# reidprichard/ORC

Measured on AMD Instinct MI355X. Metric: SIMPLE iterations/s (10.24M-cell hex channel equivalents; = iterations/s at N=1), higher is better.
Workload: dtype f64

## Files before the change

include/orc_amd.h:

```cpp
#ifndef ORC_AMD_H
#define ORC_AMD_H

#include <stdint.h>
#include "orc_types.h"

#ifdef __cplusplus
extern "C" {
#endif

typedef struct OrcMesh OrcMesh;
typedef struct OrcSolver OrcSolver;

int orc_init(int device_ordinal);
int orc_device_count(void);
int orc_synchronize(void);
const char *orc_status_string(int status);
const char *orc_last_error(void);
int orc_reload_environment(void);
int orc_device_memory(int64_t *free_bytes, int64_t *total_bytes);
int orc_device_info(char *buf, int cap);
void orc_settings_default(OrcSettings *s);

OrcMesh *orc_mesh_create(int64_t n_cells, int64_t n_faces, int32_t n_zones,
                         const int64_t *face_c0, const int64_t *face_c1, const int32_t *face_zone,
                         const double *face_area, const double *face_normal , const double *face_centroid ,
                         const double *cell_centroid , const double *cell_volume,
                         const int64_t *cell_face_ptr , const int64_t *cell_faces,
                         const int32_t *zone_type, const double *zone_scalar, const double *zone_vector ,
                         int *status);
OrcMesh *orc_mesh_create_reordered(int64_t n_cells, int64_t n_faces, int32_t n_zones,
                                   const int64_t *face_c0, const int64_t *face_c1, const int32_t *face_zone,
                                   const double *face_area, const double *face_normal, const double *face_centroid,
                                   const double *cell_centroid, const double *cell_volume,
                                   const int64_t *cell_face_ptr, const int64_t *cell_faces,
                                   const int32_t *zone_type, const double *zone_scalar, const double *zone_vector,
                                   int32_t ordering, int *status);
int orc_mesh_cell_order(const OrcMesh *m, int64_t *global_ids );
OrcMesh *orc_mesh_create_partitioned(int64_t n_owned, int64_t n_cells, int64_t n_cells_global, int64_t n_faces, int32_t n_zones,
                                     const int64_t *face_c0, const int64_t *face_c1, const int32_t *face_zone, const double *face_area,
                                     const double *face_normal, const double *face_centroid, const double *cell_centroid,
                                     const double *cell_volume, const int64_t *cell_face_ptr, const int64_t *cell_faces,
                                     const int32_t *zone_type, const double *zone_scalar, const double *zone_vector, int32_t n_peers,
                                     const int32_t *peers, const int64_t *send_ptr, const int64_t *send_idx, const int64_t *recv_ptr,
                                     int *status);
int64_t orc_mesh_n_owned(const OrcMesh *m);
typedef struct OrcPartition OrcPartition;
OrcPartition *orc_mesh_partition(int64_t n_cells, int64_t n_faces, const int64_t *face_c0, const int64_t *face_c1, const int32_t *face_zone,
                                 const double *face_area, const double *face_normal, const double *face_centroid,
                                 const double *cell_centroid, const double *cell_volume, const int64_t *cell_face_ptr,
                                 const int64_t *cell_faces, int32_t n_ranks, int32_t rank, int32_t ordering, int *status);
OrcPartition *orc_mesh_partition_owner(int64_t n_cells, int64_t n_faces, const int64_t *face_c0, const int64_t *face_c1, const int32_t *face_zone,
                                       const double *face_area, const double *face_normal, const double *face_centroid,
                                       const double *cell_centroid, const double *cell_volume, const int64_t *cell_face_ptr,
                                       const int64_t *cell_faces, const int32_t *cell_owner, int32_t n_ranks, int32_t rank, int64_t n_global,
                                       int *status);
void orc_partition_destroy(OrcPartition *p);
int orc_partition_sizes(const OrcPartition *p, int64_t *n_owned, int64_t *n_local, int64_t *n_global, int64_t *n_faces, int64_t *n_cell_faces,
                        int32_t *n_peers, int64_t *n_send);
int orc_partition_arrays(const OrcPartition *p, int64_t *face_c0, int64_t *face_c1, int32_t *face_zone, double *face_area, double *face_normal,
                         double *face_centroid, double *cell_centroid, double *cell_volume, int64_t *cell_face_ptr, int64_t *cell_faces,
                         int64_t *global_ids, int64_t *global_face_ids, int32_t *peers, int64_t *send_ptr, int64_t *send_idx, int64_t *recv_ptr);
OrcMesh *orc_partition_upload(const OrcPartition *p, int32_t n_zones, const int32_t *zone_type, const double *zone_scalar,
                              const double *zone_vector, int *status);
int orc_mesh_update_zones(OrcMesh *m, const int32_t *zone_type, const double *zone_scalar, const double *zone_vector);
void orc_mesh_destroy(OrcMesh *m);
int64_t orc_mesh_n_cells(const OrcMesh *m);
int64_t orc_mesh_nnz(const OrcMesh *m);
int orc_mesh_matrix_pattern(const OrcMesh *m, int64_t *row_ptr , int64_t *col_idx );

typedef struct OrcMeshData OrcMeshData;
OrcMeshData *orc_read_mesh(const char *mesh_path, int *status);
void orc_mesh_data_destroy(OrcMeshData *d);
int orc_mesh_data_sizes(const OrcMeshData *d, int32_t *dimensions, int64_t *n_vertices, int64_t *n_cells, int64_t *n_faces,
                        int64_t *n_cell_faces, int64_t *n_face_nodes, int32_t *n_zones);
int orc_mesh_data_arrays(const OrcMeshData *d, int64_t *face_c0, int64_t *face_c1, int32_t *face_zone, double *face_area,
                         double *face_normal, double *face_centroid, double *cell_centroid, double *cell_volume,
                         int64_t *cell_face_ptr, int64_t *cell_faces);
int orc_mesh_data_nodes(const OrcMeshData *d, double *vertices , int64_t *face_node_ptr , int64_t *face_nodes);
int orc_mesh_data_zone(const OrcMeshData *d, int32_t k, uint64_t *zone_id, int32_t *zone_type, double *scalar_value,
                       double *vector_value , char *name, int64_t name_len);
int orc_mesh_data_zone_index(const OrcMeshData *d, const char *name);
int orc_mesh_data_set_zone(OrcMeshData *d, const char *name, int32_t zone_type, double scalar_value, const double *vector_value );
OrcMesh *orc_mesh_upload(const OrcMeshData *d, int *status);
int orc_mesh_sync_zones(OrcMesh *m, const OrcMeshData *d);

int orc_write_data(const char *output_file_name, int64_t n_cells, const double *cell_centroid , const double *u,
                   const double *v, const double *w, const double *p, int decimal_precision);
int orc_read_data(const char *data_file_path, int64_t capacity, double *u, double *v, double *w, double *p, int64_t *n_read);
int orc_write_gradients(const OrcMesh *m, const double *cell_centroid, const double *u, const double *v, const double *w,
                        const double *p, const char *output_file_name, int decimal_precision, const OrcSettings *settings);

int orc_iterative_solve(int64_t n, const int64_t *row_ptr, const int64_t *col_idx, const double *values,
                        const double *b, double *solution_vector , uint64_t iteration_count,
                        int method , double relaxation_factor, double convergence_threshold,
                        int preconditioner );
int orc_iterative_solve3(int64_t n, const int64_t *row_ptr, const int64_t *col_idx, const double *const values[3],
                         const double *const b[3], double *const solution_vectors[3] , uint64_t iteration_count,
                         int method, double relaxation_factor, double convergence_threshold, int preconditioner,
                         int status_out[3]);
int orc_set_breakdown_guard(int on);
int64_t orc_breakdown_guard_events(int reset);
int orc_set_reduction_order(int order);
int64_t orc_last_jacobi_sweeps(void);
int orc_set_gmres_restart(int m);
int orc_last_gmres_stats(int64_t *steps, int64_t *cycles, double *initial_residual, double *final_estimate);
int orc_csr_spmv(int64_t n, const int64_t *row_ptr, const int64_t *col_idx, const double *values, const double *x,
                 double *y, int reps, double *avg_ms);

int orc_amg_coarsen(int64_t n, const int64_t *row_ptr, const int64_t *col_idx, const double *values, int64_t *partner ,
                    int64_t *out_n_coarse, int64_t *out_nnz, int64_t *out_row_ptr, int64_t *out_col, double *out_val,
                    int *rounds);

int orc_debug_coloring(int64_t n, const int64_t *row_ptr, const int64_t *col_idx, int32_t *colors , int32_t *n_colors);

int orc_build_momentum_diffusion_matrix(const OrcMesh *m, int diffusion_scheme, double mu,
                                        double *a_values , double *b_u, double *b_v, double *b_w);
int orc_initialize_momentum_matrix(const OrcMesh *m, double *a_values );
int orc_build_momentum_advection_matrices(const OrcMesh *m, double *a_u_values, double *a_v_values, double *a_w_values,
                                          double *b_u, double *b_v, double *b_w, const double *a_di_values,
                                          const double *u, const double *v, const double *w, const double *p,
                                          const OrcSettings *settings, double rho, double peclet[3]);
int orc_build_pressure_correction_matrices(const OrcMesh *m, const double *u, const double *v, const double *w,
                                           const double *p, const double *a_u_values, const double *a_v_values,
                                           const double *a_w_values, const OrcSettings *settings, double rho,
                                           double *a_values , double *b );

int orc_calculate_gradients(const OrcMesh *m, const double *u, const double *v, const double *w, const double *p,
                            const OrcSettings *settings, double *grad_p, double *grad_u);
int orc_check_boundary_conditions(const OrcMesh *m, int *constraint_type);
int orc_initialize_pressure_field(const OrcMesh *m, double *p );
int orc_initialize_flow(const OrcMesh *m, double mu, double rho, uint64_t iteration_count, const OrcSettings *settings,
                        double *u, double *v, double *w, double *p);
int orc_initialize_velocity_field(const OrcMesh *m, const OrcSettings *settings, double *u, double *v, double *w, double *psi);
int orc_initialize_flow_new(const OrcMesh *m, double mu, double rho, uint64_t iteration_count,
                            double *u, double *v, double *w, double *p);
typedef void (*OrcReportFn)(uint64_t iteration, const double mean_velocity[3], const double peclet[3],
                            double velocity_correction, double pressure_correction, double ms_per_iter, void *user);
int orc_solve_steady(OrcMesh *m, double *u, double *v, double *w, double *p, const OrcSettings *settings,
                     double rho, double mu, uint64_t iteration_count, uint64_t reporting_interval,
                     OrcReportFn report_cb, void *user);

OrcSolver *orc_solver_create(OrcMesh *m, const OrcSettings *settings, double rho, double mu, int *status);
void orc_solver_destroy(OrcSolver *s);
int orc_solver_set_fields(OrcSolver *s, const double *u, const double *v, const double *w, const double *p);
int orc_solver_get_fields(OrcSolver *s, double *u, double *v, double *w, double *p);
int orc_solver_iterate(OrcSolver *s, uint64_t iterations, double *report);
int orc_solver_snapshot(OrcSolver *s);
int orc_solver_restore(OrcSolver *s);
int orc_solver_assemble_momentum(OrcSolver *s, double *a_u, double *a_v, double *a_w, double *b_u, double *b_v, double *b_w, double peclet[3]);
int orc_solver_assemble_pressure(OrcSolver *s, double *a_p, double *b_p);

int orc_bench_spmv(OrcSolver *s, int reps, double *avg_ms, double *checksum);
int orc_bench_bicgstab_iteration(OrcSolver *s, int reps, double *avg_ms);
int orc_bench_inloop_products(OrcSolver *s, int reps, double avg_ms[4]);
const char *orc_bench_inloop_variant(void);
int orc_bench_gs_sweep(OrcSolver *s, int reps, double *avg_ms, int *n_colors);
int orc_bench_gs_sweep0(OrcSolver *s, int reps, double avg_ms[2], int *n_colors);
int orc_bench_amg_levels(OrcSolver *s, int reps, int64_t *rows, int64_t *nnz, int64_t *padded, double *avg_ms, int *n_levels);
long long orc_debug_halo_overlaps(void);
int orc_debug_stream_report(char *buf, int cap);
int orc_debug_amg_coarse_product(int64_t n, const int64_t *row_ptr, const int64_t *col_idx, const double *values, int scaled, const double *x,
                                 double *y, int *has_window_mirror);
long long orc_debug_collectives(int reset);
int orc_debug_clamp_partials_grid(long long requested);
int orc_debug_max_partials(void);
int orc_debug_amg_certification(long long out[2], int reset);
int orc_debug_xwin_counters(long long out[3], int reset);
long long orc_debug_shared_galerkin(int reset);
int orc_profile_enable(int on);
int orc_profile_report(char *buf, int64_t buf_len);

int orc_hex_channel_sizes(int64_t nx, int64_t ny, int64_t nz, int64_t *n_cells, int64_t *n_faces, int64_t *n_cell_faces);
int orc_hex_channel_generate(int64_t nx, int64_t ny, int64_t nz, double lx, double ly, double lz,
                             int64_t *face_c0, int64_t *face_c1, int32_t *face_zone, double *face_area,
                             double *face_normal, double *face_centroid, double *cell_centroid, double *cell_volume,
                             int64_t *cell_face_ptr, int64_t *cell_faces);
int orc_hex_channel_write_msh(const char *path, int64_t nx, int64_t ny, int64_t nz, double lx, double ly, double lz);

int orc_mixed_channel_write_msh(const char *path, int64_t nx, int64_t ny, int64_t nz, double lx, double ly, double lz,
                                int64_t *n_cells, int64_t *n_faces);
int orc_poly_channel_write_msh(const char *path, int64_t nx, int64_t ny, int64_t nz, double lx, double ly, double lz,
                               int64_t *n_cells, int64_t *n_faces);
OrcMeshData *orc_mixed_channel_generate(int64_t nx, int64_t ny, int64_t nz, double lx, double ly, double lz, int polyhedra, int *status);

#define ORC_COMM_ID_BYTES 128
int orc_comm_get_unique_id(unsigned char id[ORC_COMM_ID_BYTES]);
int orc_comm_init(const unsigned char id[ORC_COMM_ID_BYTES], int rank, int world_size);
int orc_comm_finalize(void);
int orc_comm_selftest(void);
int orc_comm_init_self_loop(void);
int orc_comm_set_host_transport(void *exchange_fn, void *allreduce_fn, void *user);

#ifdef __cplusplus
}
#endif
#endif
```

orc_amd/csrc/amg.hip:

```cpp
#include <algorithm>
#include <array>
#include <atomic>
#include <chrono>
#include <cmath>
#include <mutex>

#include <thread>

#include "linalg_kernels.hpp"

namespace orc {


__device__ __forceinline__ int64_t sell_pos(const SellDev &P, int64_t row, int k) { return P.slice_ptr[row >> 6] + (int64_t)k * 64 + (row & 63); }

struct AggCounters {
    int changed;
    int rounds;
};

__global__ void agg_reset_k(int *__restrict__ taken_by, int64_t n) {
    for (int64_t i = (int64_t)blockIdx.x * blockDim.x + threadIdx.x; i < n; i += (int64_t)gridDim.x * blockDim.x) taken_by[i] = 0x7fffffff;
}
__global__ void agg_scatter_k(const int *__restrict__ choice, int *__restrict__ taken_by, int64_t n) {
// ... 361 lines not shown
            const int a = (e >= b1) + (e >= b2) + (e >= b3);
            const int c = src_col[e];
            const int own_base = a == 0 ? 0 : (a == 1 ? b1 : (a == 2 ? b2 : b3));
            int rank = e - own_base;
            if (a != 0 && b1 > 0) rank += lds_upper_bound(src_col, b1, c);
            if (a != 1 && b2 > b1) rank += a > 1 ? lds_upper_bound(src_col + b1, b2 - b1, c) : lds_lower_bound(src_col + b1, b2 - b1, c);
            if (a != 2 && b3 > b2) rank += a > 2 ? lds_upper_bound(src_col + b2, b3 - b2, c) : lds_lower_bound(src_col + b2, b3 - b2, c);
            if (a != 3 && b4 > b3) rank += lds_lower_bound(src_col + b3, b4 - b3, c);
            m_col[rank] = c;
            m_val[rank] = src_val[e];
#pragma unroll
            for (int x = 0; x < kX; ++x) x_m[(size_t)x * h + rank] = x_src[(size_t)x * h + e];
        }
        __syncthreads();
        int cntT = 0;
        for (int b0 = 0; b0 < cnt; b0 += G) {
            const int e = b0 + lane;
            int head = 0;
            if (e < cnt) head = (e == 0) || (m_col[e] != m_col[e - 1]);
            int tot;
            const int slot = cntT + group_excl_scan<G>(head, tot);
            if (head) {
                const int j = m_col[e];
                double acc = 0. + m_val[e];
                double xacc[kX > 0 ? kX : 1];
#pragma unroll
                for (int x = 0; x < kX; ++x) xacc[x] = 0. + x_m[(size_t)x * h + e];
                for (int q = e + 1; q < cnt && m_col[q] == j; ++q) {
                    acc += m_val[q];
#pragma unroll
                    for (int x = 0; x < kX; ++x) xacc[x] += x_m[(size_t)x * h + q];
                }
                src_col[slot] = j;
                src_val[slot] = acc;
#pragma unroll
                for (int x = 0; x < kX; ++x) x_src[(size_t)x * h + slot] = xacc[x];
            }
            cntT += tot;
        }
        __syncthreads();
        const int pair0_n = (active_n && 2 * I_n < n_fine) ? choice[2 * I_n] : -1;
        const int pair1_n = (active_n && 2 * I_n + 1 < n_fine) ? choice[2 * I_n + 1] : -1;
        const int *tj = src_col;
        const double *tv = src_val;
        int nU = 0;
        for (int b0 = 0; b0 < cntT; b0 += G) {
            const int e = b0 + lane;
            int k0 = -1, k1 = -1;
            if (e < cntT) {
                const int j = tj[e];
                const int cj = choice[j], mj = chooser[j];
                if (cj >= 0) {
                    const bool dup = (j & 1) && e > 0 && tj[e - 1] == j - 1 && choice[j - 1] >= 0;
                    if (!dup) k0 = j >> 1;
                }
                if (mj >= 0) {
                    const int Jp = mj >> 1;
                    bool drop = cj >= 0 && Jp == (j >> 1);
                    if (!drop) {
                        const int p = lds_lower_bound(tj, cntT, 2 * Jp);
                        const bool has_even = p < cntT && tj[p] == 2 * Jp;
                        if (has_even && choice[2 * Jp] >= 0) drop = true;
                        else {
                            const int q = has_even ? p + 1 : p;
                            if (q < cntT && tj[q] == 2 * Jp + 1 && choice[2 * Jp + 1] >= 0) drop = true;
                        }
                    }
                    if (!drop) {
                        const int sib = mj ^ 1;
                        if (sib < n_fine) {
                            const int js = choice[sib];
                            if (js >= 0 && js < j) {
                                const int p = lds_lower_bound(tj, cntT, js);
                                if (p < cntT && tj[p] == js) drop = true;
                            }
                        }
                    }
                    if (!drop) k1 = Jp;
                }
            }
            int tot;
            int slot = nU + group_excl_scan<G>((k0 >= 0 ? 1 : 0) + (k1 >= 0 ? 1 : 0), tot);
            if (k0 >= 0) U[slot++] = k0;
            if (k1 >= 0) U[slot] = k1;
            nU += tot;
        }
        __syncthreads();
        const long long off = active ? slice_base[I >> 6] + intra_off[I] : 0;
        for (int e = lane; e < nU; e += G) {
            const int u = U[e];
            int rank = 0;
            for (int q = 0; q < nU; ++q) rank += U[q] < u ? 1 : 0;
            const RRow RJ = restriction_row(choice, u, A.P.n);
            double acc = 0.;
            double xacc[kX > 0 ? kX : 1];
#pragma unroll
            for (int x = 0; x < kX; ++x) xacc[x] = 0.;
#pragma unroll
            for (int a = 0; a < 4; ++a) {
                if (a < RJ.n) {
                    const int p = lds_lower_bound(tj, cntT, RJ.idx[a]);
                    if (p < cntT && tj[p] == RJ.idx[a]) {
                        acc += tv[p] * RJ.w[a];
#pragma unroll
                        for (int x = 0; x < kX; ++x) xacc[x] += x_src[(size_t)x * h + p] * RJ.w[a];
                    }
                }
            }
            s_col[off + rank] = u;
            s_val[off + rank] = acc;
#pragma unroll
            for (int x = 0; x < kX; ++x) X.s_val[x][off + rank] = xacc[x];
        }
        if (active && lane == 0) row_len_c[I] = nU;
        __syncthreads();
        active = active_n; I = I_n; pair0 = pair0_n; pair1 = pair1_n;
    }
}

constexpr int kPackDepth = 16;
template <bool kValuesOnly = false>
__global__ __launch_bounds__(64) void galerkin_pack_fused_k(SellDev Pc, const long long *__restrict__ slice_base, const int *__restrict__ intra_off,
                                                            const int *__restrict__ s_col, const double *__restrict__ s_val, int *__restrict__ col_c,
                                                            double *__restrict__ val_c, int *__restrict__ diag_c, const int64_t *__restrict__ pk_ptr,
                                                            int *__restrict__ pk_col, double *__restrict__ pk_val) {
    __shared__ int t_col[kPackDepth * 65];
    __shared__ double t_val[kPackDepth * 65];
    const int lane = threadIdx.x;
    const int kk = lane & (kPackDepth - 1), rr = lane / kPackDepth;
    for (int64_t slice = blockIdx.x; slice < Pc.n_slices; slice += gridDim.x) {
        const int64_t I = slice * 64 + lane;
        const bool live = I < Pc.n;
        const int len = live ? Pc.row_len[I] : 0;
        const long long src = live ? slice_base[slice] + intra_off[I] : 0;
        const int src_lo = (int)(unsigned)(src & 0xffffffffll), src_hi = (int)(src >> 32);
        const int64_t base = Pc.slice_ptr[slice];
        const int width = (int)((Pc.slice_ptr[slice + 1] - base) >> 6);
        int64_t pk_off = pk_ptr ? pk_ptr[slice] : 0;
        int d = -1;
        for (int kc = 0; kc < width; kc += kPackDepth) {
#pragma unroll 4
            for (int rb = 0; rb < 64 / (64 / kPackDepth); ++rb) {
                const int row = rb * (64 / kPackDepth) + rr;
                const int rlen = __shfl(len, row, 64);
                const long long rsrc = ((long long)__shfl(src_hi, row, 64) << 32) | (long long)(unsigned)__shfl(src_lo, row, 64);
                const int k = kc + kk;
                if (k < rlen) {
                    if (!kValuesOnly) t_col[kk * 65 + row] = s_col[rsrc + k];
                    t_val[kk * 65 + row] = s_val[rsrc + k];
                }
            }
            __syncthreads();
            const int kend = min(kPackDepth, width - kc);
            for (int q = 0; q < kend; ++q) {
                const int k = kc + q;
                const bool in = k < len;
                const int c = (in && !kValuesOnly) ? t_col[q * 65 + lane] : (int)I;
                const double v = in ? t_val[q * 65 + lane] : 0.;
                const int64_t pos = base + (int64_t)k * 64 + lane;
                if (live) {
                    if (!kValuesOnly) col_c[pos] = c;
                    val_c[pos] = v;
                    if (!kValuesOnly && in && c == (int)I) d = (int)pos;
                }
                if (pk_ptr) {
                    const unsigned long long m = __ballot(in);
                    const int rank = __builtin_amdgcn_mbcnt_hi((unsigned)(m >> 32), __builtin_amdgcn_mbcnt_lo((unsigned)m, 0u));
                    if (in) {
                        if (!kValuesOnly) pk_col[pk_off + rank] = c;
                        pk_val[pk_off + rank] = v;
                    }
                    pk_off += __popcll(m);
                }
            }
            __syncthreads();
        }
        if (live && !kValuesOnly) diag_c[I] = d;
    }
}

constexpr int kGalerkinTiers = 7;
constexpr int kBoundIters = 32;
__global__ __launch_bounds__(64) void galerkin_bound_k(SellDev P, const int *__restrict__ choice, int64_t n_coarse, int *__restrict__ out_max,
                                                       unsigned long long *__restrict__ out_sum, int *__restrict__ intra_off,
                                                       long long *__restrict__ slice_tot, int *__restrict__ tier_count, int *__restrict__ tier_list, int min_tier) {
    __shared__ signed char tiers[kBoundIters][64];
    const int lane = threadIdx.x;
    const int64_t n_slices = (n_coarse + 63) / 64;
    int mx = 0;
    unsigned long long sm = 0;
    int cnt[kGalerkinTiers];
#pragma unroll
    for (int t = 0; t < kGalerkinTiers; ++t) cnt[t] = 0;
    const int64_t per_wave = (n_slices + gridDim.x - 1) / gridDim.x;
    const int64_t s_lo = (int64_t)blockIdx.x * per_wave, s_hi = s_lo + per_wave < n_slices ? s_lo + per_wave : n_slices;
    int it = 0;
    for (int64_t s = s_lo; s < s_hi && it < kBoundIters; ++s, ++it) {
        const int64_t I = s * 64 + lane;
        int c = 0;
        if (I < n_coarse) {
            const RRow R = restriction_row(choice, I, P.n);
#pragma unroll
            for (int a = 0; a < 4; ++a)
                if (a < R.n) c += P.row_len[R.idx[a]];
        }
        int tot;
        const int ex = wave_excl_scan(2 * c, tot);
        if (I < n_coarse) intra_off[I] = ex;
        if (lane == 0) slice_tot[s] = tot;
        mx = max(mx, c);
        sm += (unsigned long long)c;
        int tier = -1;
        if (I < n_coarse) {
            tier = min_tier;
            while (tier < kGalerkinTiers - 1 && (64 << tier) < 2 * c) ++tier;
        }
        tiers[it][lane] = (signed char)tier;
#pragma unroll
        for (int t = 0; t < kGalerkinTiers; ++t) cnt[t] += __popcll(__ballot(tier == t));
    }
    int base[kGalerkinTiers];
#pragma unroll
    for (int t = 0; t < kGalerkinTiers; ++t) {
        base[t] = 0;
        if (cnt[t] > 0) {
            if (lane == 0) base[t] = atomicAdd(&tier_count[t], cnt[t]);
            base[t] = __shfl(base[t], 0, 64);
        }
    }
    it = 0;
    for (int64_t s = s_lo; s < s_hi && it < kBoundIters; ++s, ++it) {
        const int64_t I = s * 64 + lane;
        const int tier = tiers[it][lane];
#pragma unroll
        for (int t = 0; t < kGalerkinTiers; ++t) {
            const unsigned long long m = __ballot(tier == t);
            if (m == 0ull) continue;
            if (tier == t) tier_list[(int64_t)t * n_coarse + base[t] + __popcll(m & ((1ull << lane) - 1ull))] = (int)I;
            base[t] += __popcll(m);
        }
    }
#pragma unroll
    for (int off = 32; off > 0; off >>= 1) {
        mx = max(mx, __shfl_down(mx, off, 64));
        sm += __shfl_down(sm, off, 64);
    }
    if (lane == 0) { atomicMax(out_max, mx); atomicAdd(out_sum, sm); }
}

constexpr int kScanThreads = 256;
__device__ __forceinline__ long long block_excl_scan(long long v, long long *buf , long long &total) {
    const int t = threadIdx.x;
    buf[t] = v;
    __syncthreads();
    for (int off = 1; off < kScanThreads; off <<= 1) {
        const long long x = t >= off ? buf[t - off] : 0;
        __syncthreads();
        buf[t] += x;
        __syncthreads();
    }
    total = buf[kScanThreads - 1];
    const long long r = buf[t] - v;
    __syncthreads();
    return r;
}

__global__ __launch_bounds__(kBlock) void slice_sizes_k(const int *__restrict__ row_len, int64_t n, int n_slices, int64_t *__restrict__ w_sell,
                                                        int64_t *__restrict__ w_pk) {
    const int lane = threadIdx.x & 63;
    const int64_t wave = ((int64_t)blockIdx.x * blockDim.x + threadIdx.x) >> 6, waves = ((int64_t)gridDim.x * blockDim.x) >> 6;
    for (int64_t s = wave; s < n_slices; s += waves) {
        const int64_t r = s * 64 + lane;
        const int len = r < n ? row_len[r] : 0;
        int mx = len, sum = len;
#pragma unroll
        for (int off = 32; off > 0; off >>= 1) {
            mx = max(mx, __shfl_xor(mx, off, 64));
            sum += __shfl_xor(sum, off, 64);
        }
        if (lane == 0) { w_sell[s] = (int64_t)mx * 64; w_pk[s] = ((int64_t)sum + 15) & ~(int64_t)15; }
    }
}
constexpr int kScanBlocks = 128;
__global__ __launch_bounds__(kScanThreads) void scan_part_k(const long long *__restrict__ in_a, const long long *__restrict__ in_b, int64_t n, int64_t chunk,
                                                            long long *__restrict__ part ) {
    __shared__ long long buf[kScanThreads];
    const int64_t lo = (int64_t)blockIdx.x * chunk, hi = std::min<int64_t>(n, lo + chunk);
    long long sa = 0, sb = 0;
    for (int64_t e = lo + threadIdx.x; e < hi; e += kScanThreads) { sa += in_a[e]; if (in_b) sb += in_b[e]; }
    long long ta, tb;
    (void)block_excl_scan(sa, buf, ta);
    (void)block_excl_scan(sb, buf, tb);
    if (threadIdx.x == 0) { part[blockIdx.x] = ta; part[kScanBlocks + blockIdx.x] = tb; }
}
__global__ __launch_bounds__(kScanThreads) void scan_mid_k(long long *__restrict__ part, int n_blocks) {
    __shared__ long long buf[kScanThreads];
    const int t = threadIdx.x;
    const long long va = t < n_blocks ? part[t] : 0, vb = t < n_blocks ? part[kScanBlocks + t] : 0;
    long long ta, tb;
    const long long ra = block_excl_scan(va, buf, ta);
    const long long rb = block_excl_scan(vb, buf, tb);
    if (t < n_blocks) { part[t] = ra; part[kScanBlocks + t] = rb; }
    if (t == 0) { part[2 * kScanBlocks] = ta; part[2 * kScanBlocks + 1] = tb; }
}
__global__ __launch_bounds__(kScanThreads) void scan_write_k(const long long *__restrict__ in_a, const long long *__restrict__ in_b, int64_t n, int64_t chunk,
                                                             const long long *__restrict__ part, long long *__restrict__ out_a, long long *__restrict__ out_b,
                                                             int write_totals ) {
    __shared__ long long buf[kScanThreads];
    const int64_t lo = (int64_t)blockIdx.x * chunk, hi = std::min<int64_t>(n, lo + chunk);
    long long base_a = part[blockIdx.x], base_b = part[kScanBlocks + blockIdx.x];
    for (int64_t t0 = lo; t0 < hi; t0 += kScanThreads) {
        const int64_t e = t0 + threadIdx.x;
        const long long va = e < hi ? in_a[e] : 0, vb = (in_b && e < hi) ? in_b[e] : 0;
        long long ta, tb = 0;
        const long long ra = block_excl_scan(va, buf, ta);
        long long rb = 0;
        if (in_b) rb = block_excl_scan(vb, buf, tb);
        if (e < hi) { out_a[e] = base_a + ra; if (in_b) out_b[e] = base_b + rb; }
        base_a += ta;
        base_b += tb;
    }
    if (write_totals && blockIdx.x == 0 && threadIdx.x == 0) { out_a[n] = part[2 * kScanBlocks]; if (in_b) out_b[n] = part[2 * kScanBlocks + 1]; }
}
static int scan_excl_dev(const long long *in_a, const long long *in_b, int64_t n, long long *out_a, long long *out_b, bool write_totals, long long *part, hipStream_t st) {
    const int64_t n1 = std::max<int64_t>(n, 1);
    int64_t chunk = (n1 + kScanBlocks - 1) / kScanBlocks;
    chunk = ((chunk + kScanThreads - 1) / kScanThreads) * kScanThreads;
    const int n_blocks = (int)((n1 + chunk - 1) / chunk);
    hipLaunchKernelGGL(scan_part_k, dim3(n_blocks), dim3(kScanThreads), 0, st, in_a, in_b, n, chunk, part);
    hipLaunchKernelGGL(scan_mid_k, dim3(1), dim3(kScanThreads), 0, st, part, n_blocks);
    hipLaunchKernelGGL(scan_write_k, dim3(n_blocks), dim3(kScanThreads), 0, st, in_a, in_b, n, chunk, (const long long *)part, out_a, out_b, write_totals ? 1 : 0);
    ORC_HIP(hipGetLastError());
    return ORC_OK;
}


constexpr int kXBitWords = 8192;
__device__ unsigned long long g_xwin_counters[3];
constexpr int kXBitWordsSmall = 4096;
template <int kWords, bool kSecond>
__global__ __launch_bounds__(kBlock) void xwin_build_k(SellDev P, PackedDev pk, int *__restrict__ wcol, int *__restrict__ wsize,
                                                       unsigned short *__restrict__ lidx, int64_t n_blocks, int win_cap, int bit_words, int pass_words,
                                                       int *__restrict__ pending ) {
    if (kSecond && *pending == 0) return;
    __shared__ unsigned bits[kWords];
    __shared__ unsigned short wpre[kWords];
    __shared__ int s_min, s_max, s_part[kBlock];
    const int tid = threadIdx.x, lane = tid & 63, wave = tid >> 6;
    unsigned long long n_built = 0, n_capped = 0, n_spanned = 0;
    for (int64_t b = blockIdx.x; b < n_blocks; b += gridDim.x) {
        if (kSecond && wsize[b] != -2) continue;
        const int64_t row = b * kXWinRows + tid;
        const bool live = row < P.n;
        const int len = live ? P.row_len[row] : 0;
        const int64_t rbase = live ? P.slice_ptr[row >> 6] + (row & 63) : 0;
        if (tid == 0) { s_min = 0x7fffffff; s_max = -1; }
        __syncthreads();
        if (len > 0) {
            atomicMin(&s_min, P.col[rbase]);
            atomicMax(&s_max, P.col[rbase + (int64_t)(len - 1) * 64]);
        }
        __syncthreads();
        const int cmin = s_min, span = s_max - s_min + 1;
        const int words = (span + 31) >> 5;
        if (s_max < 0) {
            if (tid == 0) wsize[b] = 0;
            __syncthreads();
            continue;
        }
        if (!kSecond && words <= bit_words && words > pass_words) {
            if (tid == 0) { wsize[b] = -2; atomicAdd(pending, 1); }
            __syncthreads();
            continue;
        }
        ++n_built;
        if (words > bit_words || words > kWords) {
            if (tid == 0) wsize[b] = -1;
            ++n_spanned;
            __syncthreads();
            continue;
        }
        for (int w = tid; w < words; w += kBlock) bits[w] = 0u;
        __syncthreads();
        for (int k = 0; k < len; ++k) {
            const int c = P.col[rbase + (int64_t)k * 64] - cmin;
            atomicOr(&bits[c >> 5], 1u << (c & 31));
        }
        __syncthreads();
        const int per = (words + kBlock - 1) / kBlock;
        int local = 0;
        for (int w = tid * per; w < words && w < (tid + 1) * per; ++w) local += __popc(bits[w]);
        s_part[tid] = local;
        __syncthreads();
        for (int off = 1; off < kBlock; off <<= 1) {
            const int t = tid >= off ? s_part[tid - off] : 0;
            __syncthreads();
            s_part[tid] += t;
            __syncthreads();
        }
        const int total = s_part[kBlock - 1];
        if (total > win_cap) {
            __syncthreads();
            if (tid == 0) wsize[b] = -1;
            ++n_capped;
            __syncthreads();
            continue;
        }
        int run = s_part[tid] - local;
        int *wc = wcol + b * kXWinCap;
        for (int w = tid * per; w < words && w < (tid + 1) * per; ++w) {
            wpre[w] = (unsigned short)run;
            unsigned m = bits[w];
            while (m) {
                const int bit = __ffs(m) - 1;
                wc[run++] = cmin + (w << 5) + bit;
                m &= m - 1;
            }
        }
        if (tid == 0) wsize[b] = total;
        __syncthreads();
        const int64_t slice = b * 4 + wave;
        if (slice < P.n_slices) {
            const int64_t sbase = P.slice_ptr[slice];
            const int width = (int)((P.slice_ptr[slice + 1] - sbase) >> 6);
            int64_t off = pk.ptr[slice];
            for (int q = 0; q < width; ++q) {
                const bool in = q < len;
                const unsigned long long m = __ballot(in);
                const int rank = __builtin_amdgcn_mbcnt_hi((unsigned)(m >> 32), __builtin_amdgcn_mbcnt_lo((unsigned)m, 0u));
                if (in) {
                    const int c = P.col[sbase + (int64_t)q * 64 + lane] - cmin;
                    lidx[off + rank] = (unsigned short)(wpre[c >> 5] + __popc(bits[c >> 5] & ((1u << (c & 31)) - 1u)));
                }
                off += __popcll(m);
            }
        }
        __syncthreads();
    }
    if (tid == 0) {
        if (n_built) atomicAdd(&g_xwin_counters[0], n_built);
        if (n_capped) atomicAdd(&g_xwin_counters[1], n_capped);
        if (n_spanned) atomicAdd(&g_xwin_counters[2], n_spanned);
    }
}

constexpr int kXWinCapSizes = 5;
__device__ __constant__ int kXWinCapSizeDev[kXWinCapSizes] = {2048, 2560, 3200, 4000, kXWinCap};
static const int kXWinCapSize[kXWinCapSizes] = {2048, 2560, 3200, 4000, kXWinCap};
__global__ __launch_bounds__(kBlock) void xwin_cap_k(const int *__restrict__ wsize, int64_t n_blocks, int *__restrict__ over) {
    int c[kXWinCapSizes] = {0, 0, 0, 0, 0};
    for (int64_t b = (int64_t)blockIdx.x * blockDim.x + threadIdx.x; b < n_blocks; b += (int64_t)gridDim.x * blockDim.x) {
        const int ws = wsize[b];
#pragma unroll
        for (int q = 0; q < kXWinCapSizes; ++q) c[q] += ws > kXWinCapSizeDev[q] ? 1 : 0;
    }
#pragma unroll
    for (int q = 0; q < kXWinCapSizes; ++q)
        if (c[q]) atomicAdd(over + q, c[q]);
}

__global__ __launch_bounds__(kBlock) void xwin_stats_k(const int *__restrict__ wcol, const int *__restrict__ wsize, int64_t n_blocks, unsigned long long *__restrict__ out) {
    for (int64_t b = blockIdx.x; b < n_blocks; b += gridDim.x) {
        const int ws = wsize[b];
        if (ws <= 0) { if (threadIdx.x == 0 && ws < 0) atomicAdd(out + 4, 1ull); continue; }
        const int *wc = wcol + b * kXWinCap;
        unsigned long long runs = 0, long_entries = 0;
        for (int j = threadIdx.x; j < ws; j += kBlock) {
            if (j == 0 || wc[j] != wc[j - 1] + 1) {
                ++runs;
                int e = j + 1;
                while (e < ws && wc[e] == wc[e - 1] + 1) ++e;
                if (e - j >= 8) long_entries += (unsigned long long)(e - j);
            }
        }
        atomicAdd(out + 1, runs);
        atomicAdd(out + 2, long_entries);
        if (threadIdx.x == 0) {
            atomicAdd(out + 0, (unsigned long long)ws);
            if (wc[ws - 1] - wc[0] < 65536) atomicAdd(out + 3, 1ull);
        }
    }
}

__global__ __launch_bounds__(64) void narrow_build_k(SellDev P, unsigned short *__restrict__ col16, int *__restrict__ colbase, int *__restrict__ too_wide) {
    const int lane = threadIdx.x;
    for (int64_t slice = blockIdx.x; slice < P.n_slices; slice += gridDim.x) {
        const int64_t row = slice * 64 + lane;
        const int64_t sb = P.slice_ptr[slice];
        const int width = (int)((P.slice_ptr[slice + 1] - sb) >> 6);
        const int len = row < P.n ? P.row_len[row] : 0;
        for (int k = 0; k < width; ++k) {
            const bool in = k < len;
            const int c = in ? P.col[sb + (int64_t)k * 64 + lane] : 0;
            int lo = in ? c : 0x7fffffff, hi = in ? c : -1;
#pragma unroll
            for (int off = 32; off > 0; off >>= 1) {
                lo = min(lo, __shfl_xor(lo, off, 64));
                hi = max(hi, __shfl_xor(hi, off, 64));
            }
            if (hi < 0) lo = 0;
            if (lane == 0) {
                colbase[(sb >> 6) + k] = lo;
                if (hi >= 0 && hi - lo > 65535) atomicOr(too_wide, 1);
            }
            col16[sb + (int64_t)k * 64 + lane] = in ? (unsigned short)(c - lo) : (unsigned short)0;
        }
    }
}

__global__ void nan_to_status_k(const double *__restrict__ value, int *status, int code) {
    if (threadIdx.x == 0 && blockIdx.x == 0 && isnan(value[0])) atomicCAS(status, 0, code);
}

struct CoarseLevel {
    SellDev P;
    double *val = nullptr;
    PackedDev pk;
    XWinDev xw;
    RowsDev rows;
    bool rows_transient = false;
    int64_t n = 0, padded = 0;
    int *choice = nullptr, *chooser = nullptr;
    int rounds = 0;
};

__global__ void agg_verify_k(MatView A, const int *__restrict__ choice, const int *__restrict__ taken_by, AggCounters *C) {
    int bad = 0;
    for (int64_t i = (int64_t)blockIdx.x * blockDim.x + threadIdx.x; i < A.P.n; i += (int64_t)gridDim.x * blockDim.x)
        if (agg_eval_row(A, taken_by, i, true) != choice[i]) ++bad;
    if (bad) atomicAdd(&C->changed, bad);
}

struct DaCounters {
    int overflow;
    int steps;
    int list;
    int scans;
    int longest;
};

__device__ __forceinline__ int da_peek(const int *holder, int j) { return __hip_atomic_load(holder + j, __ATOMIC_RELAXED, __HIP_MEMORY_SCOPE_AGENT); }

__global__ __launch_bounds__(kBlock) void da_first_k(MatView A, int *holder, int2 *__restrict__ list, DaCounters *C, int *__restrict__ prefs) {
    const int64_t i = (int64_t)blockIdx.x * blockDim.x + threadIdx.x;
    int loser = -1, lost_on = -1;
    if (i < A.P.n) {
        const int len = A.P.row_len[i];
        const int64_t base = A.P.slice_ptr[i >> 6] + (i & 63);
        double bv[kPrefs];
        int bj[kPrefs];
#pragma unroll
        for (int q = 0; q < kPrefs; ++q) { bv[q] = 1.7976931348623157e308; bj[q] = -1; }
        double best = 1.7976931348623157e308;
        int fj = -1, cand = 0;
        for (int k = 0; k < len; ++k) {
            const int64_t pos = base + (int64_t)k * 64;
            const int j = A.P.col[pos];
            if (j == i || j >= A.P.n) continue;
            const double a = view_value(A, i, pos);
            if (!(a < 1.7976931348623157e308)) continue;
            ++cand;
            int pos_q = kPrefs;
#pragma unroll
            for (int q = kPrefs - 1; q >= 0; --q)
                if (a < bv[q]) pos_q = q;
#pragma unroll
            for (int q = kPrefs - 1; q >= 1; --q)
                if (q > pos_q) { bv[q] = bv[q - 1]; bj[q] = bj[q - 1]; }
#pragma unroll
            for (int q = 0; q < kPrefs; ++q)
                if (q == pos_q) { bv[q] = a; bj[q] = j; }
            if (!(a < best)) continue;
            if (da_peek(holder, j) < (int)i) continue;
            best = a; fj = j;
        }
        int4 pl;
        pl.x = bj[0]; pl.y = bj[1]; pl.z = bj[2];
        pl.w = (cand > kPrefs && bj[3] >= 0) ? (bj[3] | kPrefMore) : bj[3];
        reinterpret_cast<int4 *>(prefs)[i] = pl;
        if (fj >= 0) {
            const int old = atomicMin(&holder[fj], (int)i);
            if (old < (int)i) { loser = (int)i; lost_on = fj; }
            else if (old != 0x7fffffff) { loser = old; lost_on = fj; }
        }
    }
    const int slot = wave_append_slot(&C->list, loser >= 0);
    if (loser >= 0) list[slot] = make_int2(loser, lost_on);
// ... 431 lines not shown
        }
        const int excl = incl - len;
        if (live) new_intra[row] = excl;
        const long long ob = old_base[slice];
        const int64_t nb = new_base[slice];
        const int oi = live ? old_intra[row] : 0;
        for (int r = 0; r < 64; ++r) {
            const int n = __shfl(len, r, 64);
            const long long src = ob + __shfl(oi, r, 64);
            const int64_t dst = nb + __shfl(excl, r, 64);
            for (int e = lane; e < n; e += 64) {
                out_col[dst + e] = s_col[src + e];
                out_val[dst + e] = s_val[src + e];
            }
        }
    }
}

struct GalerkinSibling {
    const MatView *A = nullptr;
    Arena *arena = nullptr;
    Arena *rows_arena = nullptr;
    CoarseLevel *L = nullptr;
};
static std::atomic<long long> g_shared_galerkin{0};
long long debug_shared_galerkin(bool reset) {
    const long long v = g_shared_galerkin.load(std::memory_order_relaxed);
    if (reset) g_shared_galerkin.store(0, std::memory_order_relaxed);
    return v;
}

static int galerkin(const MatView &A, const int *choice, const int *chooser, Arena &arena, CoarseLevel &L, Arena *scratch = nullptr, bool last_level = false,
                    const GalerkinSibling *sib = nullptr, int n_sib = 0) {
    if (n_sib < 0 || n_sib > 2 || (n_sib > 0 && (!scratch || !sib))) return set_error(ORC_ERR_BAD_ARGUMENT, "galerkin: bad sibling arguments");
    Arena &tmp = scratch ? *scratch : arena;
    ArenaScope tmp_scope(tmp);
    const int64_t n = A.P.n, nc = n / 2 + n % 2;
    hipStream_t st = ctx().stream;
    int *row_len, *diag, *flags, *intra_off;
    long long *slice_tot, *slice_base;
    unsigned long long *counters;
    int64_t *slice_ptr;
    const int n_slices = (int)((nc + 63) / 64);
    const size_t ncs = (size_t)std::max<int64_t>(nc, 1);
    const bool trace_t = cfg().amg_trace;
    double t_mark = 0.;
    auto lap = [&](const char *what) {
        if (!trace_t) return;
        (void)hipStreamSynchronize(st);
        const double now = std::chrono::duration<double, std::milli>(std::chrono::steady_clock::now().time_since_epoch()).count();
        if (what) fprintf(stderr, "[amg phase n=%lld] %s %.3f ms\n", (long long)n, what, now - t_mark);
        t_mark = now;
    };
    lap(nullptr);
    ORC_TRY(arena.alloc(ncs, &row_len));
    ORC_TRY(arena.alloc(ncs, &diag));
    ORC_TRY(tmp.alloc(ncs, &intra_off));
    ORC_TRY(tmp.alloc((size_t)n_slices + 1, &slice_tot));
    ORC_TRY(tmp.alloc((size_t)n_slices + 1, &slice_base));
    ORC_TRY(arena.alloc((size_t)n_slices + 1, &slice_ptr));
    ORC_TRY(tmp.alloc((size_t)4, &flags));
    ORC_TRY(tmp.alloc((size_t)2, &counters));
    ORC_HIP(hipMemsetAsync(flags, 0, 4 * sizeof(int), st));
    ORC_HIP(hipMemsetAsync(counters, 0, 2 * sizeof(unsigned long long), st));
    const std::array<int, kGalerkinTiers> tier_group = [] {
        std::array<int, kGalerkinTiers> g = {16, 16, 32, 64, 64, 64, 64};
        if (!cfg().galerkin_groups.empty()) {
            const char *e = cfg().galerkin_groups.c_str();
            int t = 0;
            for (const char *q = e; *q && t < kGalerkinTiers; ++t) {
                const int v = atoi(q);
                if (v == 16 || v == 32 || v == 64) g[t] = v;
                while (*q && *q != ',') ++q;
                if (*q == ',') ++q;
            }
        }
        return g;
    }();
    int *tier_count, *tier_list;
    ORC_TRY(tmp.alloc((size_t)kGalerkinTiers + 1, &tier_count));
    ORC_TRY(tmp.alloc((size_t)kGalerkinTiers * ncs, &tier_list));
    ORC_HIP(hipMemsetAsync(tier_count, 0, (kGalerkinTiers + 1) * sizeof(int), st));
    const int64_t bound_grid = std::max<int64_t>(std::min<int64_t>(std::max<int64_t>(n_slices, 1), 8192), ((int64_t)n_slices + kBoundIters - 1) / kBoundIters);
    hipLaunchKernelGGL(galerkin_bound_k, dim3((unsigned)bound_grid), dim3(64), 0, st, A.P, choice, nc, flags, counters + 1, intra_off,
                       slice_tot, tier_count, tier_list, 0);
    long long *scan_part;
    ORC_TRY(tmp.alloc((size_t)2 * kScanBlocks + 2, &scan_part));
    ORC_TRY(scan_excl_dev(slice_tot, nullptr, (int64_t)n_slices, slice_base, nullptr, false, scan_part, st));
    int hflags[4];
    unsigned long long hcount[2];
    ORC_HIP(hipMemcpyAsync(hflags, flags, sizeof(hflags), hipMemcpyDeviceToHost, st));
    int htier[kGalerkinTiers];
    ORC_HIP(hipMemcpyAsync(hcount, counters, sizeof(hcount), hipMemcpyDeviceToHost, st));
    ORC_HIP(hipMemcpyAsync(htier, tier_count, sizeof(htier), hipMemcpyDeviceToHost, st));
    ORC_HIP(hipStreamSynchronize(st));
    const int max_cand = std::max(hflags[0], 1);
    const long long scratch_cap = (long long)std::max<unsigned long long>(2ull * hcount[1], 64ull);
    int *s_col;
    double *s_val;
    ORC_TRY(tmp.alloc((size_t)scratch_cap, &s_col));
    ORC_TRY(tmp.alloc((size_t)scratch_cap, &s_val));
    MergeSiblings X;
    const bool fine_mirror = A.rows.col != nullptr;
    for (int x = 0; x < n_sib; ++x) {
        const MatView &B = *sib[x].A;
        if (B.P.n != n || B.P.col != A.P.col || (B.rows.col != nullptr) != fine_mirror || (fine_mirror && B.rows.col != A.rows.col))
            return set_error(ORC_ERR_BAD_ARGUMENT, "galerkin: a sibling system does not share the leader's pattern");
        X.val[x] = fine_mirror ? B.rows.val : B.val;
        X.s1[x] = B.s1;
        X.s2[x] = B.s2;
        ORC_TRY(tmp.alloc((size_t)scratch_cap, &X.s_val[x]));
    }
    lap("galerkin bounds");
    static std::once_flag attr_once;
    std::call_once(attr_once, [] {
        (void)hipFuncSetAttribute(reinterpret_cast<const void *>(&galerkin_merge_k<64, 1>), hipFuncAttributeMaxDynamicSharedMemorySize, 160 * 1024);
        (void)hipFuncSetAttribute(reinterpret_cast<const void *>(&galerkin_merge_k<64, 2>), hipFuncAttributeMaxDynamicSharedMemorySize, 160 * 1024);
        (void)hipFuncSetAttribute(reinterpret_cast<const void *>(&galerkin_merge_k<64, 3>), hipFuncAttributeMaxDynamicSharedMemorySize, 160 * 1024);
        (void)hipFuncSetAttribute(reinterpret_cast<const void *>(&galerkin_merge_k<32, 2>), hipFuncAttributeMaxDynamicSharedMemorySize, 160 * 1024);
        (void)hipFuncSetAttribute(reinterpret_cast<const void *>(&galerkin_merge_k<32, 3>), hipFuncAttributeMaxDynamicSharedMemorySize, 160 * 1024);
        (void)hipFuncSetAttribute(reinterpret_cast<const void *>(&galerkin_merge_k<16, 2>), hipFuncAttributeMaxDynamicSharedMemorySize, 160 * 1024);
        (void)hipFuncSetAttribute(reinterpret_cast<const void *>(&galerkin_merge_k<16, 3>), hipFuncAttributeMaxDynamicSharedMemorySize, 160 * 1024);
    });
    if ((size_t)2 * max_cand > (size_t)(64 << (kGalerkinTiers - 1))) return set_error(ORC_ERR_BAD_ARGUMENT, "Galerkin row too long for LDS (%d candidates)", max_cand);
    for (int t = 0; t < kGalerkinTiers; ++t) {
        if (htier[t] == 0) continue;
        const int cap = 64 << t;
        int G = tier_group[t];
        while (G < 64 && (size_t)cap * (size_t)(12 + 8 * n_sib) * (size_t)(64 / G) > (size_t)150 * 1024) G <<= 1;
        const int rows_per_wave = 64 / G;
        const size_t smem = (size_t)cap * (size_t)(12 + 8 * n_sib) * (size_t)rows_per_wave;
        if (smem > (size_t)160 * 1024) return set_error(ORC_ERR_BAD_ARGUMENT, "Galerkin row too long for a shared pass (%d candidates, %d systems)", max_cand, n_sib + 1);
        const int merge_waves = n_sib == 0 ? 24 : 16;
        const int waves_per_cu = (int)std::max<size_t>(1, std::min<size_t>((size_t)merge_waves, (size_t)(150 * 1024) / smem));
        const int g = (int)std::min<int64_t>(((int64_t)htier[t] + rows_per_wave - 1) / rows_per_wave, (int64_t)256 * waves_per_cu);
        const int *tl = tier_list + (int64_t)t * nc, *tc = tier_count + t;
#define ORC_MERGE(GG, NS) hipLaunchKernelGGL(HIP_KERNEL_NAME(galerkin_merge_k<GG, NS>), dim3(g), dim3(64), smem, st, A, choice, chooser, nc, cap, row_len, slice_base, intra_off, s_col, s_val, tl, tc, X)
        if (n_sib == 0) {
            if (G == 16) ORC_MERGE(16, 1);
            else if (G == 32) ORC_MERGE(32, 1);
            else ORC_MERGE(64, 1);
        } else if (n_sib == 1) {
            if (G == 16) ORC_MERGE(16, 2);
            else if (G == 32) ORC_MERGE(32, 2);
            else ORC_MERGE(64, 2);
        } else {
            if (G == 16) ORC_MERGE(16, 3);
            else if (G == 32) ORC_MERGE(32, 3);
            else ORC_MERGE(64, 3);
        }
#undef ORC_MERGE
    }
    lap("galerkin product");
    int64_t *pk_ptr, *w_sell, *w_pk;
    ORC_TRY(arena.alloc((size_t)n_slices + 1, &pk_ptr));
    ORC_TRY(tmp.alloc((size_t)n_slices + 1, &w_sell));
    ORC_TRY(tmp.alloc((size_t)n_slices + 1, &w_pk));
    hipLaunchKernelGGL(slice_sizes_k, dim3((unsigned)std::min<int64_t>(((int64_t)n_slices + 3) / 4, 4096)), dim3(kBlock), 0, st, row_len, nc, n_slices, w_sell, w_pk);
    static_assert(sizeof(long long) == sizeof(int64_t), "64-bit tables");
    ORC_TRY(scan_excl_dev(reinterpret_cast<const long long *>(w_sell), reinterpret_cast<const long long *>(w_pk), (int64_t)n_slices, reinterpret_cast<long long *>(slice_ptr),
                          reinterpret_cast<long long *>(pk_ptr), true, scan_part, st));
    ORC_HIP(hipGetLastError());
    int64_t padded = 0, packed_total = 0;
    ORC_HIP(hipMemcpyAsync(&packed_total, pk_ptr + n_slices, sizeof(int64_t), hipMemcpyDeviceToHost, st));
    ORC_HIP(hipMemcpyAsync(&padded, slice_ptr + n_slices, sizeof(int64_t), hipMemcpyDeviceToHost, st));
    ORC_HIP(hipMemcpyAsync(hflags, flags, sizeof(hflags), hipMemcpyDeviceToHost, st));
    ORC_HIP(hipStreamSynchronize(st));
    if (hflags[1]) return set_error(ORC_ERR_BAD_ARGUMENT, "Galerkin overflow (%d)", hflags[1]);
    if (padded >= ((int64_t)1 << 31)) return set_error(ORC_ERR_BAD_ARGUMENT, "coarse matrix too large for 32-bit offsets");
    int *col;
    double *val;
    ORC_TRY(arena.alloc((size_t)std::max<int64_t>(padded, 1), &col));
    ORC_TRY(arena.alloc((size_t)std::max<int64_t>(padded, 1), &val));
    SellDev Pc;
    Pc.n = nc; Pc.ncols = nc; Pc.n_slices = n_slices; Pc.ragged = padded < 24 * nc ? 2 : 1; Pc.padded = padded; Pc.slice_ptr = slice_ptr; Pc.row_len = row_len; Pc.col = col; Pc.diag_pos = diag;
    const int xwin_min = cfg().spmv_xwin_min_nnz;
    const bool long_rows = packed_total >= (int64_t)xwin_min * nc;
    const bool ragged_rows = 2 * packed_total >= (int64_t)xwin_min * nc && (double)padded >= 1.15 * (double)packed_total;
    const bool mirror = xwin_min >= 0 && packed_total > 0 && (long_rows || ragged_rows);
    int *pk_col = nullptr;
    double *pk_val = nullptr;
    if (mirror) {
        ORC_TRY(arena.alloc((size_t)packed_total, &pk_col));
        ORC_TRY(arena.alloc((size_t)packed_total, &pk_val));
    }
    hipLaunchKernelGGL(galerkin_pack_fused_k<false>, dim3((unsigned)std::max<int64_t>(1, std::min<int64_t>(n_slices, 256 * 12))), dim3(64), 0, st, Pc, slice_base, intra_off,
                       s_col, s_val, col, val, diag, mirror ? (const int64_t *)pk_ptr : (const int64_t *)nullptr, pk_col, pk_val);
    ORC_HIP(hipGetLastError());
    double *x_val[2] = {nullptr, nullptr}, *x_pk_val[2] = {nullptr, nullptr};
    for (int x = 0; x < n_sib; ++x) {
        ORC_TRY(sib[x].arena->alloc((size_t)std::max<int64_t>(padded, 1), &x_val[x]));
        if (mirror) ORC_TRY(sib[x].arena->alloc((size_t)packed_total, &x_pk_val[x]));
        hipLaunchKernelGGL(galerkin_pack_fused_k<true>, dim3((unsigned)std::max<int64_t>(1, std::min<int64_t>(n_slices, 256 * 12))), dim3(64), 0, st, Pc, slice_base, intra_off,
                           s_col, (const double *)X.s_val[x], (int *)nullptr, x_val[x], (int *)nullptr, mirror ? (const int64_t *)pk_ptr : (const int64_t *)nullptr, (int *)nullptr,
                           x_pk_val[x]);
        ORC_HIP(hipGetLastError());
    }
    lap("galerkin pack");
    const bool narrow_on = cfg().spmv_narrow_cols;
    if (narrow_on && !mirror && padded > 0) {
        unsigned short *c16;
        int *cbase, *wide;
        ORC_TRY(arena.alloc((size_t)padded, &c16));
        ORC_TRY(arena.alloc((size_t)(padded / 64) + 1, &cbase));
        ORC_TRY(tmp.alloc((size_t)1, &wide));
        ORC_HIP(hipMemsetAsync(wide, 0, sizeof(int), st));
        hipLaunchKernelGGL(narrow_build_k, dim3((unsigned)std::max<int64_t>(1, std::min<int64_t>(n_slices, 256 * 32))), dim3(64), 0, st, Pc, c16, cbase, wide);
        ORC_HIP(hipGetLastError());
        int h_wide = 1;
        ORC_HIP(hipMemcpyAsync(&h_wide, wide, sizeof(int), hipMemcpyDeviceToHost, st));
        ORC_HIP(hipStreamSynchronize(st));
        if (!h_wide) { Pc.col16 = c16; Pc.colbase = cbase; }
    }
    L.P = Pc; L.val = val; L.n = nc; L.padded = padded;
    L.pk = PackedDev();
    L.xw = XWinDev();
    L.rows = RowsDev();
    for (int x = 0; x < n_sib; ++x) {
        CoarseLevel &Lx = *sib[x].L;
        Lx = CoarseLevel();
        Lx.P = Pc; Lx.val = x_val[x]; Lx.n = nc; Lx.padded = padded; Lx.rounds = L.rounds;
        Lx.choice = L.choice; Lx.chooser = L.chooser;
    }
    if (!scratch) { L.rows.slice_base = slice_base; L.rows.intra_off = intra_off; L.rows.col = s_col; L.rows.val = s_val; }
    if (scratch && packed_total > 0 && !last_level) {
        Arena &rows_arena = scratch->companion();
        rows_arena.release(Arena::Mark{0, 0});
        int *r_col, *r_intra;
        double *r_val;
        ORC_TRY(rows_arena.alloc((size_t)packed_total, &r_col));
        ORC_TRY(rows_arena.alloc((size_t)packed_total, &r_val));
        ORC_TRY(rows_arena.alloc(ncs, &r_intra));
        L.rows_transient = true;
        hipLaunchKernelGGL(rows_compact_k, dim3((unsigned)std::max<int64_t>(1, std::min<int64_t>(n_slices, 256 * 16))), dim3(64), 0, st, (const int *)row_len, nc, n_slices,
                           (const long long *)slice_base, (const int *)intra_off, (const int *)s_col, (const double *)s_val, (const int64_t *)pk_ptr, r_intra, r_col, r_val);
        ORC_HIP(hipGetLastError());
        L.rows.slice_base = reinterpret_cast<const long long *>(pk_ptr); L.rows.intra_off = r_intra; L.rows.col = r_col; L.rows.val = r_val;
        for (int x = 0; x < n_sib; ++x) {
            Arena &xa = sib[x].rows_arena ? *sib[x].rows_arena : *sib[x].arena;
            if (sib[x].rows_arena) xa.release(Arena::Mark{0, 0});
            int *xr_col, *xr_intra;
            double *xr_val;
            ORC_TRY(xa.alloc((size_t)packed_total, &xr_col));
            ORC_TRY(xa.alloc((size_t)packed_total, &xr_val));
            ORC_TRY(xa.alloc(ncs, &xr_intra));
            hipLaunchKernelGGL(rows_compact_k, dim3((unsigned)std::max<int64_t>(1, std::min<int64_t>(n_slices, 256 * 16))), dim3(64), 0, st, (const int *)row_len, nc, n_slices,
                               (const long long *)slice_base, (const int *)intra_off, (const int *)s_col, (const double *)X.s_val[x], (const int64_t *)pk_ptr, xr_intra, xr_col, xr_val);
            ORC_HIP(hipGetLastError());
            CoarseLevel &Lx = *sib[x].L;
            Lx.rows.slice_base = reinterpret_cast<const long long *>(pk_ptr); Lx.rows.intra_off = xr_intra; Lx.rows.col = xr_col; Lx.rows.val = xr_val;
            Lx.rows_transient = sib[x].rows_arena != nullptr;
        }
    }
    if (mirror) {
        L.pk.ptr = pk_ptr; L.pk.col = pk_col; L.pk.val = pk_val; L.pk.total = packed_total;
        const int64_t n_blocks = ((int64_t)n_slices + 3) / 4;
        int *wcol, *wsize;
        unsigned short *lidx;
        ORC_TRY(arena.alloc((size_t)n_blocks * kXWinCap, &wcol));
        ORC_TRY(arena.alloc((size_t)n_blocks, &wsize));
        ORC_TRY(arena.alloc((size_t)packed_total, &lidx));
        const int win_cap = cfg().xwin_cap > 0 ? std::min(kXWinCap, cfg().xwin_cap) : kXWinCap;
        const int bit_words = cfg().xwin_bitwords > 0 ? std::min(kXBitWords, cfg().xwin_bitwords) : kXBitWords;
        const int small_words = cfg().xwin_small_bitwords > 0 ? std::min(kXBitWordsSmall, cfg().xwin_small_bitwords) : kXBitWordsSmall;
        int *pending;
        ORC_TRY(tmp.alloc((size_t)1, &pending));
        ORC_HIP(hipMemsetAsync(pending, 0, sizeof(int), st));
        hipLaunchKernelGGL(HIP_KERNEL_NAME(xwin_build_k<kXBitWordsSmall, false>), dim3((unsigned)std::min<int64_t>(n_blocks, 2048)), dim3(kBlock), 0, st, Pc, L.pk, wcol, wsize, lidx,
                           n_blocks, win_cap, bit_words, small_words, pending);
        if (bit_words > small_words)
            hipLaunchKernelGGL(HIP_KERNEL_NAME(xwin_build_k<kXBitWords, true>), dim3((unsigned)std::min<int64_t>(n_blocks, 2048)), dim3(kBlock), 0, st, Pc, L.pk, wcol, wsize, lidx,
                               n_blocks, win_cap, bit_words, kXBitWords, pending);
        if (trace_t) {
            int hp = 0;
            ORC_HIP(hipMemcpyAsync(&hp, pending, sizeof(int), hipMemcpyDeviceToHost, st));
            ORC_HIP(hipStreamSynchronize(st));
            fprintf(stderr, "[amg windows n=%lld] %lld blocks, %d left to the full bitmap\n", (long long)nc, (long long)n_blocks, hp);
        }
        ORC_HIP(hipGetLastError());
        L.xw.wcol = wcol; L.xw.wsize = wsize; L.xw.lidx = lidx;
        {
            int *over;
            ORC_TRY(tmp.alloc((size_t)kXWinCapSizes, &over));
            ORC_HIP(hipMemsetAsync(over, 0, kXWinCapSizes * sizeof(int), st));
            hipLaunchKernelGGL(xwin_cap_k, dim3((unsigned)std::max<int64_t>(1, std::min<int64_t>((n_blocks + kBlock - 1) / kBlock, 64))), dim3(kBlock), 0, st, (const int *)wsize, n_blocks, over);
            int h_over[kXWinCapSizes];
            ORC_HIP(hipMemcpyAsync(h_over, over, sizeof(h_over), hipMemcpyDeviceToHost, st));
            ORC_HIP(hipStreamSynchronize(st));
            int cap = win_cap;
            for (int q = 0; q < kXWinCapSizes && cfg().xwin_level_cap; ++q)
                if (kXWinCapSize[q] <= win_cap && (int64_t)h_over[q] * 100 <= n_blocks) { cap = kXWinCapSize[q]; break; }
            L.xw.cap = cap;
            if (trace_t) fprintf(stderr, "[amg windows n=%lld] LDS share %d entries per workgroup (%d of %lld blocks have larger windows)\n", (long long)nc, cap,
                                 cap < win_cap ? h_over[std::find(kXWinCapSize, kXWinCapSize + kXWinCapSizes, cap) - kXWinCapSize] : 0, (long long)n_blocks);
        }
        {
            const size_t n_wg = (size_t)((n_blocks + 7) / 8 * 8);
            double *fs;
            unsigned *fc;
            ORC_TRY(arena.alloc(2 * n_wg, &fs));
            ORC_TRY(arena.alloc((size_t)4, &fc));
            ORC_HIP(hipMemsetAsync(fc, 0, 4 * sizeof(unsigned), st));
            L.xw.fold_scratch = fs; L.xw.fold_counter = fc;
        }
        for (int x = 0; x < n_sib; ++x) {
            CoarseLevel &Lx = *sib[x].L;
            Lx.pk = L.pk;
            Lx.pk.val = x_pk_val[x];
            Lx.xw = L.xw;
            const size_t n_wg = (size_t)((n_blocks + 7) / 8 * 8);
            double *fs;
            unsigned *fc;
            ORC_TRY(sib[x].arena->alloc(2 * n_wg, &fs));
            ORC_TRY(sib[x].arena->alloc((size_t)4, &fc));
            ORC_HIP(hipMemsetAsync(fc, 0, 4 * sizeof(unsigned), st));
            Lx.xw.fold_scratch = fs; Lx.xw.fold_counter = fc;
        }
        const bool xwin_stats = cfg().debug_xwin;
        if (xwin_stats) {
            unsigned long long *d_st, h_st[5];
            ORC_TRY(tmp.alloc((size_t)5, &d_st));
            ORC_HIP(hipMemsetAsync(d_st, 0, sizeof(h_st), st));
            hipLaunchKernelGGL(xwin_stats_k, dim3((unsigned)std::min<int64_t>(n_blocks, 4096)), dim3(kBlock), 0, st, (const int *)wcol, (const int *)wsize, n_blocks, d_st);
            ORC_HIP(hipMemcpyAsync(h_st, d_st, sizeof(h_st), hipMemcpyDeviceToHost, st));
            ORC_HIP(hipStreamSynchronize(st));
            fprintf(stderr, "[orc xwin] rows %lld nnz %lld blocks %lld: window entries %llu (%.1f per row), runs %llu (%.1f entries per run), in runs >= 8: %.1f %%, span < 65536: %llu blocks, no window: %llu\n",
                    (long long)nc, (long long)packed_total, (long long)n_blocks, h_st[0], (double)h_st[0] / (double)nc, h_st[1], (double)h_st[0] / (double)std::max<unsigned long long>(h_st[1], 1),
                    100. * (double)h_st[2] / (double)std::max<unsigned long long>(h_st[0], 1), h_st[3], h_st[4]);
        }
    }
    lap("galerkin mirrors");
    if (!scratch) tmp_scope.mark = tmp.mark();
    if (n_sib > 0) g_shared_galerkin.fetch_add(n_sib, std::memory_order_relaxed);
    return ORC_OK;
}

struct MgParams {
    uint64_t max_levels, iters;
    int smoother, preconditioner;
    double relaxation, threshold;
};

struct StreamSwitch {
    hipStream_t saved;
    bool on;
    StreamSwitch(SolveSide *side) : saved(ctx().stream), on(side != nullptr) { if (on) ctx().stream = side->stream; }
    ~StreamSwitch() { if (on) ctx().stream = saved; }
};
static int side_wait_setup(SolveSide *side, hipStream_t setup_stream) {
    if (!side) return ORC_OK;
    ORC_HIP(hipEventRecord(side->ev_setup, setup_stream));
    ORC_HIP(hipStreamWaitEvent(side->stream, side->ev_setup, 0));
    return ORC_OK;
}
static int setup_wait_side(SolveSide *side, hipStream_t setup_stream) {
    if (!side) return ORC_OK;
    ORC_HIP(hipEventRecord(side->ev_solve, side->stream));
    ORC_HIP(hipStreamWaitEvent(setup_stream, side->ev_solve, 0));
    return ORC_OK;
}

struct SideScope {
    SolveSide *side;
    hipStream_t setup_stream;
    Arena &arena, &varena;
    Arena::Mark mk, vmk;
    bool release_varena;
    SideScope(SolveSide *sd, hipStream_t st, Arena &a, Arena &va, bool rel_v)
        : side(sd), setup_stream(st), arena(a), varena(va), mk(a.mark()), vmk(va.mark()), release_varena(rel_v) {}
    ~SideScope() {
        if (side) (void)setup_wait_side(side, setup_stream);
        if (release_varena) varena.release(vmk);
        arena.release(mk);
    }
    SideScope(const SideScope &) = delete;
    SideScope &operator=(const SideScope &) = delete;
};

static int multigrid_solve_dev(const MatView &A, const double *r, uint64_t level, const MgParams &mp, double threshold, Arena &arena,
                               SolveStats *stats, int *dev_status, double *out, double *add_to, SolveSide *side) {
    const int64_t n = A.P.n;
    hipStream_t st = ctx().stream;
    Arena &varena = side ? *side->arena : arena;
    SideScope scope(side, st, arena, varena, side != nullptr);
    auto leave = [](int code) { return code; };
    int *choice, *chooser;
    CoarseLevel L;
    const AmgHierarchy *hier = stats ? stats->hierarchy : nullptr;
    if (hier && (int)level <= hier->n_levels && (level == 1 ? hier->n_fine : hier->level[level - 2].n) == n) {
        const AmgHierarchy::Level &h = hier->level[level - 1];
        choice = h.choice; chooser = h.chooser;
        L.P = h.P; L.val = h.val; L.pk = h.pk; L.xw = h.xw; L.rows = h.rows; L.n = h.n; L.padded = h.padded; L.rounds = h.rounds;
    } else {
        ORC_TRY(arena.alloc((size_t)std::max<int64_t>(n, 1), &choice));
        ORC_TRY(arena.alloc((size_t)std::max<int64_t>(n, 1), &chooser));
        const int *warm = nullptr;
        SiblingPairing *sib = stats ? stats->sibling : nullptr;
        if (sib && stats->sibling_role == 2 && level == 1) warm = sib->wait((int)level, n, st);
        const int agg_st = aggregate(A, arena, choice, chooser, &L.rounds, warm);
        if (sib && stats->sibling_role == 1 && level == 1) {
            if (agg_st == ORC_OK) ORC_TRY(sib->publish((int)level, choice, n, st));
            sib->finish();
        }
        ORC_TRY(agg_st);
        ORC_TRY(galerkin(A, choice, chooser, arena, L));
    }
    const int64_t nc = L.n;
    if (stats && level < 8) {
        stats->amg_levels = std::max(stats->amg_levels, (int)level);
        stats->amg_rows[level] = nc;
        stats->amg_nnz[level] = L.padded;
        stats->amg_rounds[level] = L.rounds;
    }
    ORC_TRY(side_wait_setup(side, st));
    MatView Ac;
    Ac.P = L.P;
    Ac.val = L.val;
    Ac.pk = L.pk;
    Ac.xw = L.xw;
    Ac.rows = L.rows;
    Ac.symmetric = A.symmetric;
    double *r_prime, *e_prime, *partials, *scal;
    const bool shared_scaling = cfg().amg_shared_scaling && mp.smoother == ORC_SOLVER_BICGSTAB && mp.preconditioner == ORC_PRECOND_JACOBI;
    ScaledOperator scaled;
    {
        StreamSwitch sw(side);
        hipStream_t vs = ctx().stream;
        ORC_TRY(varena.alloc((size_t)std::max<int64_t>(nc, 1), &r_prime));
        ORC_TRY(varena.alloc((size_t)std::max<int64_t>(nc, 1), &e_prime));
        ORC_TRY(varena.alloc((size_t)kMaxPartials, &partials));
        ORC_TRY(varena.alloc((size_t)4, &scal));
        double *r_check = nullptr;
        if (ctx().reduction_order == ORC_REDUCTION_REFERENCE) ORC_TRY(varena.alloc((size_t)std::max<int64_t>(nc, 1), &r_check));
// ... 348 lines not shown
        return r;
    };

    if (!shared) {
        double *rk[3];
        for (int k = 0; k < 3; ++k) ORC_TRY(arena.alloc((size_t)n, &rk[k]));
        ORC_TRY(deinterleave3_dev(r3, rk[0], rk[1], rk[2], n));
        ORC_TRY(deinterleave3_dev(x3, x[0], x[1], x[2], n));
        ORC_HIP(hipEventRecord(ev_main, st));
        for (int k = 0; k < 3; ++k) {
            ORC_HIP(hipStreamWaitEvent(lanes[k].solve_stream, ev_main, 0));
            ORC_TRY(on_lane(k, [&] {
                return multigrid_coarse_part_dev(plain[k], rk[k], x[k], iteration_count, relaxation_factor, convergence_threshold, preconditioner,
                                                 *lanes[k].vec_arena, &lanes[k].stats, dev_status + k);
            }));
            ORC_HIP(hipEventRecord(ev_lane[k], lanes[k].solve_stream));
            ORC_HIP(hipStreamWaitEvent(st, ev_lane[k], 0));
        }
    } else {
        const AmgHierarchy::Level &L0 = H[0]->level[0];
        MatView3 Ac3;
        Ac3.P = L0.P;
        for (int k = 0; k < 3; ++k) Ac3.val[k] = H[k]->level[0].val;
        const size_t nc3 = (size_t)3 * (size_t)nc;
        double *r1, *e1, *partials, *norm3;
        ORC_TRY(arena.alloc(nc3, &r1));
        ORC_TRY(arena.alloc(nc3, &e1));
        ORC_TRY(arena.alloc((size_t)3 * kMaxPartials, &partials));
        ORC_TRY(arena.alloc((size_t)4, &norm3));
        const int dbg_mask = cfg().debug_sync;
        int step_no = 0;
        auto step = [&](const char *what) { if (dbg_mask & (1 << step_no)) { (void)hipStreamSynchronize(st); ORC_TRACE("arm3 level 1: %s done", what); } ++step_no; };
        const bool dbg_sync = (dbg_mask & 64) != 0;
        step("level 0");
        hipLaunchKernelGGL(restrict3_k, dim3(grid_for(nc)), dim3(kBlock), 0, st, (const int *)L0.choice, n, nc, (const double *)r3, r1);
        ORC_HIP(hipGetLastError());
        ORC_TRY(vec_fill(e1, 0., (int64_t)nc3));
        step("restriction");
        const bool shared_scaling = cfg().amg_shared_scaling && preconditioner == ORC_PRECOND_JACOBI;
        ScaledOperator3 scaled3;
        if (shared_scaling) ORC_TRY(jacobi_scaling_prepare3_dev(Ac3, iteration_count, arena, scaled3));
        ORC_TRY(shared_scaling ? bicgstab3_scaled_dev(scaled3, r1, e1, arena) : bicgstab3_dev(Ac3, r1, e1, iteration_count, preconditioner, arena));
        step("pre-smoothing");
        ORC_TRY(residual_norm2_3_dev(Ac3, r1, e1, partials, norm3));
        step("residual norm");
        hipLaunchKernelGGL(nan_to_status3_k, dim3(1), dim3(64), 0, st, (const double *)norm3, dev_status, (int)ORC_ERR_MULTIGRID_DIVERGED);
        ORC_HIP(hipGetLastError());
        for (int k = 0; k < 3; ++k) {
            lanes[k].stats.amg_levels = 1;
            lanes[k].stats.amg_rows[1] = nc;
            lanes[k].stats.amg_nnz[1] = H[k]->level[0].padded;
            lanes[k].stats.amg_rounds[1] = H[k]->level[0].rounds;
        }
        if (1 < mp.max_levels && nc > 16) {
            double *rk[3], *ck[3];
            for (int k = 0; k < 3; ++k) {
                ORC_TRY(arena.alloc((size_t)nc, &rk[k]));
                ORC_TRY(arena.alloc((size_t)nc, &ck[k]));
            }
            ORC_TRY(deinterleave3_dev(r1, rk[0], rk[1], rk[2], nc));
            ORC_HIP(hipEventRecord(ev_main, st));
            for (int k = 0; k < 3; ++k) {
                MatView Ak;
                Ak.P = H[k]->level[0].P; Ak.val = H[k]->level[0].val; Ak.pk = H[k]->level[0].pk; Ak.xw = H[k]->level[0].xw;
                Ak.rows = H[k]->level[0].rows;
                Ak.symmetric = plain[k].symmetric;
                ORC_HIP(hipStreamWaitEvent(lanes[k].solve_stream, ev_main, 0));
                ORC_TRY(on_lane(k, [&] {
                    return multigrid_solve_dev(Ak, rk[k], 2, mp, convergence_threshold, *lanes[k].vec_arena, &lanes[k].stats, dev_status + k, ck[k], nullptr, nullptr);
                }));
                ORC_HIP(hipEventRecord(ev_lane[k], lanes[k].solve_stream));
                ORC_HIP(hipStreamWaitEvent(st, ev_lane[k], 0));
            }
            if (dbg_sync) for (int k = 0; k < 3; ++k) { (void)hipStreamSynchronize(lanes[k].solve_stream); ORC_TRACE("arm3 level 1: lane %d levels 2.. done", k); }
            hipLaunchKernelGGL(vec_add3_k, dim3(grid_for(nc)), dim3(kBlock), 0, st, e1, (const double *)ck[0], (const double *)ck[1], (const double *)ck[2], nc);
            ORC_HIP(hipGetLastError());
            step("corrections added");
            ORC_TRY(shared_scaling ? bicgstab3_scaled_dev(scaled3, r1, e1, arena) : bicgstab3_dev(Ac3, r1, e1, iteration_count, preconditioner, arena));
            step("post-smoothing");
        }
        hipLaunchKernelGGL(prolong3_k, dim3(grid_for(n)), dim3(kBlock), 0, st, (const int *)L0.choice, (const int *)L0.chooser, n, (const double *)e1, x3);
        ORC_HIP(hipGetLastError());
        ORC_TRY(deinterleave3_dev(x3, x[0], x[1], x[2], n));
    }
    int h[4] = {0, 0, 0, 0};
    ORC_TRACE("arm3: coarse parts queued; waiting for the status words");
    ORC_HIP(hipMemcpyAsync(h, dev_status, sizeof(h), hipMemcpyDeviceToHost, st));
    ORC_HIP(hipStreamSynchronize(st));
    ORC_TRACE("arm3: done (%d %d %d)", h[0], h[1], h[2]);
    for (int k = 0; k < 3; ++k) status_out[k] = h[k];
    return ORC_OK;
}

}

namespace orc {

int amg_debug_coarsen(const MatView &A, Arena &arena, std::vector<int> &choice_h, std::vector<int64_t> &row_ptr_h,
                      std::vector<int64_t> &col_h, std::vector<double> &val_h, int *rounds, const double *x_h, double *y_h, int scaled, int *mirror_out) {
    const int64_t n = A.P.n;
    hipStream_t st = ctx().stream;
    Arena::Mark mk = arena.mark();
    int *choice, *chooser;
    ORC_TRY(arena.alloc((size_t)std::max<int64_t>(n, 1), &choice));
    ORC_TRY(arena.alloc((size_t)std::max<int64_t>(n, 1), &chooser));
    CoarseLevel L;
    ORC_TRY(aggregate(A, arena, choice, chooser, &L.rounds));
    if (rounds) *rounds = L.rounds;
    ORC_TRY(galerkin(A, choice, chooser, arena, L));
    choice_h.resize((size_t)n);
    ORC_HIP(hipMemcpyAsync(choice_h.data(), choice, sizeof(int) * (size_t)n, hipMemcpyDeviceToHost, st));
    const int64_t nc = L.n;
    if (mirror_out) *mirror_out = (L.pk.ptr && L.xw.lidx) ? 1 : 0;
    if (x_h && y_h && nc > 0) {
        MatView V;
        V.P = L.P; V.val = L.val; V.pk = L.pk; V.xw = L.xw; V.symmetric = A.symmetric;
        double *x, *y, *d1;
        ORC_TRY(arena.alloc((size_t)nc, &x));
        ORC_TRY(arena.alloc((size_t)nc, &y));
        ORC_HIP(hipMemcpyAsync(x, x_h, sizeof(double) * (size_t)nc, hipMemcpyHostToDevice, st));
        if (scaled) {
            ORC_TRY(arena.alloc((size_t)nc, &d1));
            ORC_TRY(diag_inverse_dev(V, d1));
            V.s1 = d1;
            ORC_TRY(materialize_scaled_view(V, 50, arena));
        }
        ORC_TRY(spmv_dev(V, x, y));
        ORC_HIP(hipMemcpyAsync(y_h, y, sizeof(double) * (size_t)nc, hipMemcpyDeviceToHost, st));
        ORC_HIP(hipStreamSynchronize(st));
    }
    std::vector<int> row_len((size_t)nc), col((size_t)std::max<int64_t>(L.padded, 1));
    std::vector<int64_t> slice_ptr((size_t)L.P.n_slices + 1);
    std::vector<double> val((size_t)std::max<int64_t>(L.padded, 1));
    ORC_HIP(hipMemcpyAsync(row_len.data(), L.P.row_len, sizeof(int) * (size_t)nc, hipMemcpyDeviceToHost, st));
    ORC_HIP(hipMemcpyAsync(slice_ptr.data(), L.P.slice_ptr, sizeof(int64_t) * slice_ptr.size(), hipMemcpyDeviceToHost, st));
    ORC_HIP(hipMemcpyAsync(col.data(), L.P.col, sizeof(int) * (size_t)L.padded, hipMemcpyDeviceToHost, st));
    ORC_HIP(hipMemcpyAsync(val.data(), L.val, sizeof(double) * (size_t)L.padded, hipMemcpyDeviceToHost, st));
    ORC_HIP(hipStreamSynchronize(st));
    row_ptr_h.assign((size_t)nc + 1, 0);
    for (int64_t I = 0; I < nc; ++I) row_ptr_h[(size_t)I + 1] = row_ptr_h[(size_t)I] + row_len[(size_t)I];
    col_h.resize((size_t)row_ptr_h[(size_t)nc]);
    val_h.resize((size_t)row_ptr_h[(size_t)nc]);
    for (int64_t I = 0; I < nc; ++I) {
        const int64_t base = slice_ptr[(size_t)(I >> 6)] + (I & 63);
        for (int k = 0; k < row_len[(size_t)I]; ++k) {
            col_h[(size_t)(row_ptr_h[(size_t)I] + k)] = col[(size_t)(base + (int64_t)k * 64)];
            val_h[(size_t)(row_ptr_h[(size_t)I] + k)] = val[(size_t)(base + (int64_t)k * 64)];
        }
    }
    arena.release(mk);
    return ORC_OK;
}

}
```

orc_amd/csrc/api_linalg.cpp:

```cpp
#include <algorithm>

#include "linalg.hpp"

namespace orc {
int amg_debug_coarsen(const MatView &A, Arena &arena, std::vector<int> &choice_h, std::vector<int64_t> &row_ptr_h,
                      std::vector<int64_t> &col_h, std::vector<double> &val_h, int *rounds, const double *x_h = nullptr, double *y_h = nullptr,
                      int scaled = 0, int *mirror_out = nullptr);
int gs_debug_coloring(const SellDev &P, std::vector<int> &colors, int *n_colors);
static SolveStats g_last_stats;
SolveStats &last_stats() { return g_last_stats; }
}

extern "C" {

int orc_iterative_solve(int64_t n, const int64_t *row_ptr, const int64_t *col_idx, const double *values, const double *b,
                        double *solution_vector, uint64_t iteration_count, int method, double relaxation_factor,
                        double convergence_threshold, int preconditioner) {
    using namespace orc;
    ORC_TRY(ensure_init());
    if (n < 0 || !row_ptr || (!col_idx && n > 0) || (!values && n > 0) || !b || !solution_vector)
        return set_error(ORC_ERR_BAD_ARGUMENT, "null argument");
    SellMatrix pat;
    ORC_TRY(sell_from_csr_host(n, n, row_ptr, col_idx, pat));
    const size_t nn = (size_t)std::max<int64_t>(n, 1);
    DevBuf<double> csr_vals, vals, db, dx;
    ORC_TRY(csr_vals.upload(values, (size_t)pat.nnz));
    ORC_TRY(vals.alloc((size_t)std::max<int64_t>(pat.padded, 1)));
    ORC_TRY(sell_import_values(pat, csr_vals.p, vals.p));
    ORC_TRY(db.alloc(nn));
    ORC_TRY(dx.alloc(nn));
    ORC_TRY(db.upload(b, (size_t)n));
    ORC_TRY(dx.upload(solution_vector, (size_t)n));
    MatView A;
    A.P = pat.dev();
    A.val = vals.p;
    A.symmetric = pat.symmetric;
    Arena arena;
    g_last_stats = SolveStats();
    int st = iterative_solve_dev(A, db.p, dx.p, iteration_count, method, relaxation_factor, convergence_threshold, preconditioner,
                                 arena, &g_last_stats);
    int st2 = dx.download(solution_vector, (size_t)n);
    return st != ORC_OK ? st : st2;
}

int orc_iterative_solve3(int64_t n, const int64_t *row_ptr, const int64_t *col_idx, const double *const values[3], const double *const b[3],
                         double *const solution_vectors[3], uint64_t iteration_count, int method, double relaxation_factor,
                         double convergence_threshold, int preconditioner, int status_out[3]) {
    using namespace orc;
    ORC_TRY(ensure_init());
    if (n < 0 || !row_ptr || (!col_idx && n > 0) || !values || !b || !solution_vectors) return set_error(ORC_ERR_BAD_ARGUMENT, "null argument");
    if (method != ORC_SOLVER_BICGSTAB && method != ORC_SOLVER_MULTIGRID)
        return set_error(ORC_ERR_BAD_ARGUMENT, "orc_iterative_solve3: BiCGSTAB and Multigrid arms only (method %d)", method);
    SellMatrix pat;
    ORC_TRY(sell_from_csr_host(n, n, row_ptr, col_idx, pat));
    const size_t nn = (size_t)std::max<int64_t>(n, 1);
    DevBuf<double> csr_vals, vals[3], db[3], dx[3];
    MatView3 A3;
    A3.P = pat.dev();
    for (int k = 0; k < 3; ++k) {
        ORC_TRY(csr_vals.upload(values[k], (size_t)pat.nnz));
        ORC_TRY(vals[k].alloc((size_t)std::max<int64_t>(pat.padded, 1)));
        ORC_TRY(sell_import_values(pat, csr_vals.p, vals[k].p));
        ORC_HIP(hipStreamSynchronize(ctx().stream));
        ORC_TRY(db[k].alloc(nn));
        ORC_TRY(dx[k].alloc(nn));
        ORC_TRY(db[k].upload(b[k], (size_t)n));
        ORC_TRY(dx[k].upload(solution_vectors[k], (size_t)n));
        A3.val[k] = vals[k].p;
    }
    Arena arena;
    int st = ORC_OK;
    int st3[3] = {ORC_OK, ORC_OK, ORC_OK};
    if (!triple_supported()) {
        for (int k = 0; k < 3; ++k) {
            MatView A;
            A.P = pat.dev();
            A.val = vals[k].p;
            A.symmetric = pat.symmetric;
            SolveStats stats;
            st3[k] = iterative_solve_dev(A, db[k].p, dx[k].p, iteration_count, method, relaxation_factor, convergence_threshold, preconditioner, arena, &stats);
            if (st == ORC_OK && st3[k] != ORC_OK && st3[k] != ORC_ERR_MULTIGRID_DIVERGED) st = st3[k];
        }
    } else if (method == ORC_SOLVER_BICGSTAB) {
        double *b3, *x3;
        ORC_TRY(arena.alloc(3 * nn, &b3));
        ORC_TRY(arena.alloc(3 * nn, &x3));
        ORC_TRY(interleave3_dev(db[0].p, db[1].p, db[2].p, b3, n));
        ORC_TRY(interleave3_dev(dx[0].p, dx[1].p, dx[2].p, x3, n));
        st = bicgstab3_dev(A3, b3, x3, iteration_count, preconditioner, arena);
        if (st == ORC_OK) st = deinterleave3_dev(x3, dx[0].p, dx[1].p, dx[2].p, n);
    } else {
        TripleLane lanes[3];
        Arena hier[3], vec[3], scratch[3];
        SiblingPairing sibling;
        hipStream_t streams[6] = {nullptr, nullptr, nullptr, nullptr, nullptr, nullptr};
        for (int k = 0; k < 6 && st == ORC_OK; ++k)
            st = stream_create(&streams[k], kPlainStream, k, "solve3");
        for (int k = 0; k < 3; ++k) {
            lanes[k].setup_stream = streams[2 * k]; lanes[k].solve_stream = streams[2 * k + 1];
            lanes[k].hier_arena = &hier[k]; lanes[k].vec_arena = &vec[k]; lanes[k].scratch_arena = &scratch[k];
            lanes[k].symmetric = pat.symmetric;
        }
        const double *bb[3] = {db[0].p, db[1].p, db[2].p};
        double *xx[3] = {dx[0].p, dx[1].p, dx[2].p};
        if (st == ORC_OK)
            st = multigrid_arm3_dev(A3, bb, xx, iteration_count, relaxation_factor, convergence_threshold, preconditioner, arena, lanes, &sibling, st3);
        (void)hipDeviceSynchronize();
        for (int k = 0; k < 6; ++k)
            if (streams[k]) stream_destroy(streams[k]);
    }
    for (int k = 0; k < 3; ++k) {
        const int st2 = dx[k].download(solution_vectors[k], (size_t)n);
        if (st == ORC_OK) st = st2;
        if (status_out) status_out[k] = st3[k];
    }
    if (!status_out && st == ORC_OK)
        for (int k = 0; k < 3 && st == ORC_OK; ++k) st = st3[k];
    return st;
}

int orc_csr_spmv(int64_t n, const int64_t *row_ptr, const int64_t *col_idx, const double *values, const double *x, double *y,
                 int reps, double *avg_ms) {
    using namespace orc;
    ORC_TRY(ensure_init());
    if (n < 0 || !row_ptr || !x || !y) return set_error(ORC_ERR_BAD_ARGUMENT, "null argument");
    SellMatrix pat;
    ORC_TRY(sell_from_csr_host(n, n, row_ptr, col_idx, pat));
    const size_t nn = (size_t)std::max<int64_t>(n, 1);
    DevBuf<double> csr_vals, vals, dx, dy;
    ORC_TRY(csr_vals.upload(values, (size_t)pat.nnz));
    ORC_TRY(vals.alloc((size_t)std::max<int64_t>(pat.padded, 1)));
    ORC_TRY(sell_import_values(pat, csr_vals.p, vals.p));
    ORC_TRY(dx.alloc(nn));
    ORC_TRY(dy.alloc(nn));
    ORC_TRY(dx.upload(x, (size_t)n));
    MatView A;
    A.P = pat.dev();
    A.val = vals.p;
    if (reps < 1) reps = 1;
    hipEvent_t e0, e1;
    ORC_HIP(hipEventCreate(&e0));
    ORC_HIP(hipEventCreate(&e1));
    ORC_TRY(spmv_dev(A, dx.p, dy.p));
    ORC_HIP(hipEventRecord(e0, ctx().stream));
    for (int i = 1; i < reps; ++i) ORC_TRY(spmv_dev(A, dx.p, dy.p));
    ORC_HIP(hipEventRecord(e1, ctx().stream));
    ORC_HIP(hipEventSynchronize(e1));
    float ms = 0.f;
    ORC_HIP(hipEventElapsedTime(&ms, e0, e1));
    if (avg_ms) *avg_ms = reps > 1 ? (double)ms / (reps - 1) : 0.;
    (void)hipEventDestroy(e0);
    (void)hipEventDestroy(e1);
    return dy.download(y, (size_t)n);
}

int orc_amg_coarsen(int64_t n, const int64_t *row_ptr, const int64_t *col_idx, const double *values, int64_t *partner,
                    int64_t *out_n_coarse, int64_t *out_nnz, int64_t *out_row_ptr, int64_t *out_col, double *out_val, int *rounds) {
    using namespace orc;
    ORC_TRY(ensure_init());
    SellMatrix pat;
    ORC_TRY(sell_from_csr_host(n, n, row_ptr, col_idx, pat));
    DevBuf<double> csr_vals, vals;
    ORC_TRY(csr_vals.upload(values, (size_t)pat.nnz));
    ORC_TRY(vals.alloc((size_t)std::max<int64_t>(pat.padded, 1)));
    ORC_TRY(sell_import_values(pat, csr_vals.p, vals.p));
    MatView A;
    A.P = pat.dev();
    A.val = vals.p;
    A.symmetric = pat.symmetric;
    Arena arena;
    std::vector<int> choice;
    std::vector<int64_t> rp, ci;
    std::vector<double> v;
    ORC_TRY(amg_debug_coarsen(A, arena, choice, rp, ci, v, rounds));
    if (partner) for (int64_t i = 0; i < n; ++i) partner[i] = choice[(size_t)i];
    if (out_n_coarse) *out_n_coarse = (int64_t)rp.size() - 1;
    if (out_nnz) *out_nnz = (int64_t)ci.size();
    if (out_col) {
        std::copy(rp.begin(), rp.end(), out_row_ptr);
        std::copy(ci.begin(), ci.end(), out_col);
        std::copy(v.begin(), v.end(), out_val);
    }
    return ORC_OK;
}

int orc_debug_amg_coarse_product(int64_t n, const int64_t *row_ptr, const int64_t *col_idx, const double *values, int scaled, const double *x,
                                 double *y, int *has_window_mirror) {
    using namespace orc;
    ORC_TRY(ensure_init());
    if (n < 1 || !row_ptr || !col_idx || !values || !x || !y) return set_error(ORC_ERR_BAD_ARGUMENT, "null argument");
    SellMatrix pat;
    ORC_TRY(sell_from_csr_host(n, n, row_ptr, col_idx, pat));
    DevBuf<double> csr_vals, vals;
    ORC_TRY(csr_vals.upload(values, (size_t)pat.nnz));
    ORC_TRY(vals.alloc((size_t)std::max<int64_t>(pat.padded, 1)));
    ORC_TRY(sell_import_values(pat, csr_vals.p, vals.p));
    MatView A;
    A.P = pat.dev();
    A.val = vals.p;
    A.symmetric = pat.symmetric;
    Arena arena;
    std::vector<int> choice;
    std::vector<int64_t> rp, ci;
    std::vector<double> v;
    return amg_debug_coarsen(A, arena, choice, rp, ci, v, nullptr, x, y, scaled, has_window_mirror);
}

int orc_debug_coloring(int64_t n, const int64_t *row_ptr, const int64_t *col_idx, int32_t *colors, int32_t *n_colors) {
    using namespace orc;
    ORC_TRY(ensure_init());
    SellMatrix pat;
    ORC_TRY(sell_from_csr_host(n, n, row_ptr, col_idx, pat));
    std::vector<int> c;
    int nc = 0;
    ORC_TRY(gs_debug_coloring(pat.dev(), c, &nc));
    for (int64_t i = 0; i < n; ++i) colors[i] = c[(size_t)i];
    if (n_colors) *n_colors = nc;
    return ORC_OK;
}

int64_t orc_last_jacobi_sweeps(void) { return orc::g_last_stats.jacobi_sweeps; }

int orc_set_gmres_restart(int m) {
    orc::ctx().gmres_restart = m;
    return ORC_OK;
}

int orc_last_gmres_stats(int64_t *steps, int64_t *cycles, double *initial_residual, double *final_estimate) {
    const orc::SolveStats &s = orc::g_last_stats;
    if (steps) *steps = s.gmres_steps;
    if (cycles) *cycles = s.gmres_cycles;
    if (initial_residual) *initial_residual = s.gmres_beta0;
    if (final_estimate) *final_estimate = s.gmres_estimate;
    return ORC_OK;
}

}
```

orc_amd/csrc/linalg.hip:

```cpp
#include <algorithm>
#include <atomic>
#include <cmath>
#include <cstdint>

#include "linalg_kernels.hpp"

namespace orc {


__global__ __launch_bounds__(1024) void reduce_partials_k(const double *__restrict__ partials, int count, int nq, double *__restrict__ out) {
    __shared__ double lds[16];
    for (int q = 0; q < nq; ++q) {
        double v = 0.;
        for (int i = threadIdx.x; i < count; i += blockDim.x) v += partials[(size_t)q * count + i];
        v = wave_sum(v);
        __syncthreads();
        if ((threadIdx.x & 63) == 0) lds[threadIdx.x >> 6] = v;
        __syncthreads();
        if (threadIdx.x == 0) {
            double r = 0.;
            for (int i = 0; i < (int)(blockDim.x >> 6); ++i) r += lds[i];
            out[q] = r;
        }
    }
// ... 536 lines not shown
        }
        if (blockIdx.x == 0 && threadIdx.x == 0) scal[S_FROZEN2] = 1.;
    } else {
        int64_t i = i0;
        while (i < n2) {
            const int64_t nx = i + stride;
            double2 xn = make_double2(0., 0.), pn = xn, sn = xn, tn = xn;
            if (nx < n2) { xn = x2[nx]; pn = p2[nx]; sn = s2[nx]; tn = t2[nx]; }
            const double h0 = xv.x + alpha * pv.x, h1 = xv.y + alpha * pv.y;
            x2[i] = make_double2(h0 + omega * sv.x, h1 + omega * sv.y);
            const double q0 = sv.x - omega * tv.x, q1 = sv.y - omega * tv.y;
            r2[i] = make_double2(q0, q1);
            acc += q0;
            acc += q1;
            xv = xn; pv = pn; sv = sn; tv = tn; i = nx;
        }
        if ((n & 1) && blockIdx.x == 0 && threadIdx.x == 0) {
            const int64_t i = n - 1;
            const double h = x[i] + alpha * p[i];
            const double si = s[i];
            x[i] = h + omega * si;
            const double ri = si - omega * t[i];
            r[i] = ri;
            acc += ri;
        }
    }
    const double tsum = block_sum(acc, lds);
    if (threadIdx.x == 0) partials[blockIdx.x] = tsum;
}
__global__ __launch_bounds__(kBlock) void bicg_p_k(double *__restrict__ scal, int rho_prev_idx, int rho_idx, const double *__restrict__ r,
                                                   const double *__restrict__ nu, double *__restrict__ p, int64_t n, int guard,
                                                   const double *__restrict__ fold, int fold_count) {
    __shared__ double lds16[16];
    if (bicg_frozen(scal, guard)) {
        if (guard && scal[S_FROZEN2] != 0. && blockIdx.x == 0 && threadIdx.x == 0) scal[S_FROZEN] = 1.;
        return;
    }
    const int64_t n2 = n >> 1, stride = (int64_t)gridDim.x * blockDim.x;
    double2 *p2 = reinterpret_cast<double2 *>(p);
    const double2 *r2 = reinterpret_cast<const double2 *>(r), *nu2 = reinterpret_cast<const double2 *>(nu);
    int64_t i = (int64_t)blockIdx.x * blockDim.x + threadIdx.x;
    double2 rv = make_double2(0., 0.), pv = rv, nv = rv;
    if (i < n2) { rv = r2[i]; pv = p2[i]; nv = nu2[i]; }
    double rho;
    if (fold) {
        rho = fold_partials_block(fold, fold_count, lds16);
        if (blockIdx.x == 0 && threadIdx.x == 0) scal[rho_idx] = rho;
    } else {
        rho = scal[rho_idx];
    }
    const double rho_prev = scal[rho_prev_idx];
    const double alpha = rho_prev / scal[S_SUM_NU];
    const double omega = scal[S_TS] / scal[S_TT];
    const double beta = rho / rho_prev * alpha / omega;
    if (guard && !(finite_nonzero(omega) && isfinite(beta))) {
        if (blockIdx.x == 0 && threadIdx.x == 0) scal[S_FROZEN] = 1.;
        return;
    }
    while (i < n2) {
        const int64_t nx = i + stride;
        double2 rn = make_double2(0., 0.), pn = rn, nn = rn;
        if (nx < n2) { rn = r2[nx]; pn = p2[nx]; nn = nu2[nx]; }
        p2[i] = make_double2(rv.x + beta * (pv.x - omega * nv.x), rv.y + beta * (pv.y - omega * nv.y));
        rv = rn; pv = pn; nv = nn; i = nx;
    }
    if ((n & 1) && blockIdx.x == 0 && threadIdx.x == 0) p[n - 1] = r[n - 1] + beta * (p[n - 1] - omega * nu[n - 1]);
}

__global__ void guard_event_k(const double *__restrict__ scal, int *__restrict__ counter) {
    if (scal[S_FROZEN] != 0. || scal[S_FROZEN2] != 0.) atomicAdd(counter, 1);
}

struct BicgWork {
    double *r, *p, *nu, *s, *t, *partials, *partials2, *scal;
};

static int bicg_alloc(Arena &arena, int64_t n, BicgWork &w) {
    const size_t nn = (size_t)std::max<int64_t>(n, 1);
    ORC_TRY(arena.alloc(nn, &w.r));
    ORC_TRY(arena.alloc(nn, &w.p));
    ORC_TRY(arena.alloc(nn, &w.nu));
    ORC_TRY(arena.alloc(nn, &w.s));
    ORC_TRY(arena.alloc(nn, &w.t));
    ORC_TRY(arena.alloc((size_t)2 * kMaxPartials, &w.partials));
    ORC_TRY(arena.alloc((size_t)kMaxPartials, &w.partials2));
    ORC_TRY(arena.alloc((size_t)S_COUNT, &w.scal));
    ORC_HIP(hipMemsetAsync(w.scal, 0, S_COUNT * sizeof(double), ctx().stream));
    return ORC_OK;
}

static int bicg_iteration(const MatView &A, double *x, const BicgWork &w, uint64_t it, int guard) {
    const int64_t n = A.P.n;
    const int vg = grid_for((n + 1) / 2);
    const int cur = (int)(it & 1), nxt = cur ^ 1;
    const double *skip = guard ? w.scal + S_FROZEN : nullptr;
    int g = 0;
    const bool ref = reference_order(A);
    const bool fused = !ref && A.halo == nullptr;
    ORC_TRY(launch_spmv(A, w.p, EpiStoreSum{w.nu}, w.partials, &g, skip));
    if (ref) ORC_TRY(dot_reference(nullptr, w.nu, n, w.scal + S_SUM_NU, skip));
    else if (!fused) ORC_TRY(reduce_partials(w.partials, g, 1, w.scal + S_SUM_NU, A.halo != nullptr));
    hipLaunchKernelGGL(bicg_s_k, dim3(vg), dim3(kBlock), 0, ctx().stream, w.scal, S_RHO0 + cur, w.r, w.nu, w.s, n, guard,
                       fused ? (const double *)w.partials : (const double *)nullptr, g);
    ORC_TRY(launch_spmv(A, w.s, EpiTs{w.s, w.t}, w.partials, &g, skip));
    if (ref) {
        ORC_TRY(dot_reference(w.t, w.s, n, w.scal + S_TS, skip));
        ORC_TRY(dot_reference(w.t, w.t, n, w.scal + S_TT, skip));
    } else if (!fused) ORC_TRY(reduce_partials(w.partials, g, 2, w.scal + S_TS, A.halo != nullptr));
    double *xr_partials = fused ? w.partials2 : w.partials;
    hipLaunchKernelGGL(bicg_xr_k, dim3(vg), dim3(kBlock), 0, ctx().stream, w.scal, S_RHO0 + cur, x, w.p, w.s, w.t, w.r, n, xr_partials, guard,
                       fused ? (const double *)w.partials : (const double *)nullptr, g);
    if (ref) ORC_TRY(dot_reference(nullptr, w.r, n, w.scal + S_RHO0 + nxt, skip));
    else if (!fused) ORC_TRY(reduce_partials(w.partials, vg, 1, w.scal + S_RHO0 + nxt, A.halo != nullptr));
    hipLaunchKernelGGL(bicg_p_k, dim3(vg), dim3(kBlock), 0, ctx().stream, w.scal, S_RHO0 + cur, S_RHO0 + nxt, w.r, w.nu, w.p, n, guard,
                       fused ? (const double *)w.partials2 : (const double *)nullptr, vg);
    ORC_HIP(hipGetLastError());
    return ORC_OK;
}

__global__ __launch_bounds__(kBlock) void scale_values_k(MatView A, double *__restrict__ out) {
    const int lane = threadIdx.x & 63;
    SliceWalk w(A.P.n_slices);
    for (int64_t slice = w.begin; slice < w.end; slice += w.step) {
        const int64_t row = slice * 64 + lane;
        const int64_t base = A.P.slice_ptr[slice];
        const int width = (int)((A.P.slice_ptr[slice + 1] - base) >> 6);
        const bool live = row < A.P.n;
        const double s1 = (A.s1 && live) ? A.s1[row] : 1.;
        const double s2 = (A.s2 && live) ? A.s2[row] : 1.;
        for (int k = 0; k < width; ++k) {
            const int64_t p = base + (int64_t)k * 64 + lane;
            double t = A.val[p];
            if (A.s1) t = s1 * t;
            if (A.s2) t = s2 * t;
            out[p] = t;
        }
    }
}
static inline bool materialize_scaling(uint64_t iteration_count) {
    const int min_its = cfg().materialize_scaling;
    return min_its > 0 && iteration_count >= (uint64_t)min_its;
}

__global__ __launch_bounds__(kBlock) void scale_packed_k(MatView A, double *__restrict__ out) {
    const int lane = threadIdx.x & 63;
    SliceWalk w(A.P.n_slices);
    for (int64_t slice = w.begin; slice < w.end; slice += w.step) {
        const int64_t row = slice * 64 + lane;
        const int width = (int)((A.P.slice_ptr[slice + 1] - A.P.slice_ptr[slice]) >> 6);
        const bool live = row < A.P.n;
        const int len = live ? A.P.row_len[row] : 0;
        const double s1 = (A.s1 && live) ? A.s1[row] : 1.;
        const double s2 = (A.s2 && live) ? A.s2[row] : 1.;
        int64_t off = A.pk.ptr[slice];
        for (int k = 0; k < width; ++k) {
            const bool in = k < len;
            const unsigned long long m = __ballot(in);
            const int rank = __builtin_amdgcn_mbcnt_hi((unsigned)(m >> 32), __builtin_amdgcn_mbcnt_lo((unsigned)m, 0u));
            if (in) {
                double t = A.pk.val[off + rank];
                if (A.s1) t = s1 * t;
                if (A.s2) t = s2 * t;
                out[off + rank] = t;
            }
            off += __popcll(m);
        }
    }
}

int materialize_scaled_view(MatView &A, uint64_t iteration_count, Arena &arena) {
    if (!((A.s1 || A.s2) && A.P.n > 0 && materialize_scaling(iteration_count))) return ORC_OK;
    if (A.pk.ptr) {
        if (!(A.xw.lidx && A.pk.total > 0)) return ORC_OK;
        double *scaled;
        ORC_TRY(arena.alloc((size_t)A.pk.total, &scaled));
        hipLaunchKernelGGL(scale_packed_k, dim3(spmv_grid(A.P.n_slices)), dim3(kBlock), 0, ctx().stream, A, scaled);
        ORC_HIP(hipGetLastError());
        A.pk.val = scaled;
        A.val = nullptr;
        A.s1 = A.s2 = nullptr;
        return ORC_OK;
    }
    if (A.P.padded <= 0) return ORC_OK;
    double *scaled;
    ORC_TRY(arena.alloc((size_t)A.P.padded, &scaled));
    hipLaunchKernelGGL(scale_values_k, dim3(spmv_grid(A.P.n_slices)), dim3(kBlock), 0, ctx().stream, A, scaled);
    ORC_HIP(hipGetLastError());
    A.val = scaled;
    A.s1 = A.s2 = nullptr;
    return ORC_OK;
}

static int bicgstab_run(const MatView &A, const double *b, double *x, uint64_t iteration_count, Arena &arena) {
    const int64_t n = A.P.n;
    if (n == 0) return ORC_OK;
    ArenaScope scope(arena);
    BicgWork w;
    ORC_TRY(bicg_alloc(arena, std::max(A.P.ncols, n), w));
    const int guard = ctx().breakdown_guard ? 1 : 0;
    int g = 0;
    ORC_TRY(launch_spmv(A, x, EpiResidual{b, w.r, w.p}, w.partials, &g));
    if (reference_order(A)) ORC_TRY(dot_reference(nullptr, w.r, n, w.scal + S_RHO0, nullptr));
    else ORC_TRY(reduce_partials(w.partials, g, 1, w.scal + S_RHO0, A.halo != nullptr));
    for (uint64_t it = 0; it < iteration_count; ++it) ORC_TRY(bicg_iteration(A, x, w, it, guard));
    if (guard && ctx().guard_events) {
        hipLaunchKernelGGL(guard_event_k, dim3(1), dim3(1), 0, ctx().stream, w.scal, ctx().guard_events);
        ORC_HIP(hipGetLastError());
    }
    return ORC_OK;
}

static int bicgstab_dev(const MatView &A_in, const double *b, double *x, uint64_t iteration_count, Arena &arena) {
    if (A_in.P.n == 0) return ORC_OK;
    ArenaScope scope(arena);
    MatView A = A_in;
    ORC_TRY(materialize_scaled_view(A, iteration_count, arena));
    return bicgstab_run(A, b, x, iteration_count, arena);
}

int jacobi_scaling_prepare_dev(const MatView &A_in, uint64_t iteration_count, Arena &arena, ScaledOperator &S) {
    ORC_TRY(ensure_init());
    const int64_t n = A_in.P.n;
    S = ScaledOperator();
    S.A = A_in;
    S.iterations = iteration_count;
    double *dinv;
    ORC_TRY(arena.alloc((size_t)std::max<int64_t>(n, 1), &dinv));
    if (n) {
        hipLaunchKernelGGL(diag_inverse_k, dim3(grid_for(n)), dim3(kBlock), 0, ctx().stream, A_in, dinv);
        ORC_HIP(hipGetLastError());
    }
    if (!S.A.s1) S.A.s1 = dinv;
    else if (!S.A.s2) S.A.s2 = dinv;
    else return set_error(ORC_ERR_BAD_ARGUMENT, "more than two nested Jacobi scalings");
    S.dinv = dinv;
    return materialize_scaled_view(S.A, iteration_count, arena);
}

int bicgstab_scaled_dev(const ScaledOperator &S, const double *b, double *x, Arena &arena) {
    const int64_t n = S.A.P.n;
    if (n == 0) return ORC_OK;
    ArenaScope scope(arena);
    double *b_tmp;
    ORC_TRY(arena.alloc((size_t)n, &b_tmp));
    hipLaunchKernelGGL(scale_vec_k, dim3(grid_for(n)), dim3(kBlock), 0, ctx().stream, S.dinv, b, b_tmp, n);
    ORC_HIP(hipGetLastError());
    return bicgstab_run(S.A, b_tmp, x, S.iterations, arena);
}

template <class Fn>
static int time_launches(int reps, float *ms, Fn &&launch) {
    hipEvent_t e0, e1;
    ORC_HIP(hipEventCreate(&e0));
    ORC_HIP(hipEventCreate(&e1));
    int st = launch();
    if (st == ORC_OK && hipEventRecord(e0, ctx().stream) != hipSuccess) st = set_error(ORC_ERR_HIP, "hipEventRecord failed");
    for (int i = 0; i < reps && st == ORC_OK; ++i) st = launch();
    if (st == ORC_OK && (hipEventRecord(e1, ctx().stream) != hipSuccess || hipEventSynchronize(e1) != hipSuccess)) st = set_error(ORC_ERR_HIP, "hipEventRecord failed");
    if (st == ORC_OK && hipEventElapsedTime(ms, e0, e1) != hipSuccess) st = set_error(ORC_ERR_HIP, "hipEventElapsedTime failed");
    if (st == ORC_OK) *ms /= (float)std::max(reps, 1);
    (void)hipEventDestroy(e0);
    (void)hipEventDestroy(e1);
    return st;
}
int bench_inloop_products_dev(const MatView &A, const double *x, double *y, double *partials, int reps, float ms[2]) {
    int g = 0;
    ORC_TRY(time_launches(reps, &ms[0], [&] { return launch_spmv(A, x, EpiStoreSum{y}, partials, &g, nullptr); }));
    ORC_TRY(time_launches(reps, &ms[1], [&] { return launch_spmv(A, x, EpiTs{x, y}, partials, &g, nullptr); }));
    return ORC_OK;
}

int bench_bicgstab_dev(const MatView &A, const double *b, double *x, int reps, Arena &arena, float *ms) {
    const int64_t n = A.P.n;
    Arena::Mark mk = arena.mark();
    BicgWork w;
    ORC_TRY(bicg_alloc(arena, std::max(A.P.ncols, n), w));
    int g = 0;
    ORC_TRY(launch_spmv(A, x, EpiResidual{b, w.r, w.p}, w.partials, &g));
    ORC_TRY(reduce_partials(w.partials, g, 1, w.scal + S_RHO0, A.halo != nullptr));
    hipEvent_t e0, e1;
    ORC_HIP(hipEventCreate(&e0));
    ORC_HIP(hipEventCreate(&e1));
    ORC_TRY(bicg_iteration(A, x, w, 0, 0));
    ORC_HIP(hipEventRecord(e0, ctx().stream));
    for (int it = 1; it <= reps; ++it) ORC_TRY(bicg_iteration(A, x, w, (uint64_t)it, 0));
    ORC_HIP(hipEventRecord(e1, ctx().stream));
    ORC_HIP(hipEventSynchronize(e1));
    ORC_HIP(hipEventElapsedTime(ms, e0, e1));
    *ms /= (float)reps;
    (void)hipEventDestroy(e0);
    (void)hipEventDestroy(e1);
    arena.release(mk);
    return ORC_OK;
}


bool triple_supported() { return ctx().reduction_order != ORC_REDUCTION_REFERENCE; }

struct EpiStore3 {
    static constexpr int kReductions = 0;
    double *y3;
    __device__ __forceinline__ void apply(int64_t row, const double (&acc)[3], double (&)[3][2]) const {
        reinterpret_cast<Vec3d *>(y3)[row] = Vec3d{acc[0], acc[1], acc[2]};
    }
};
struct EpiStoreSum3 {
    static constexpr int kReductions = 1;
    double *y3;
    __device__ __forceinline__ void apply(int64_t row, const double (&acc)[3], double (&red)[3][2]) const {
        reinterpret_cast<Vec3d *>(y3)[row] = Vec3d{acc[0], acc[1], acc[2]};
        red[0][0] += acc[0]; red[1][0] += acc[1]; red[2][0] += acc[2];
    }
};
struct EpiResidual3 {
    static constexpr int kReductions = 1;
    const double *b3;
    double *r3, *p3;
    __device__ __forceinline__ void apply(int64_t row, const double (&acc)[3], double (&red)[3][2]) const {
        const Vec3d b = reinterpret_cast<const Vec3d *>(b3)[row];
        const Vec3d v = {b.a - acc[0], b.b - acc[1], b.c - acc[2]};
        reinterpret_cast<Vec3d *>(r3)[row] = v;
        if (p3) reinterpret_cast<Vec3d *>(p3)[row] = v;
        red[0][0] += v.a; red[1][0] += v.b; red[2][0] += v.c;
    }
};
struct EpiResidualNorm3 {
    static constexpr int kReductions = 1;
    const double *b3;
// ... 736 lines not shown
```

orc_amd/csrc/linalg.hpp:

```cpp
#pragma once
#include <condition_variable>
#include <functional>
#include <mutex>
#include "common.hpp"
#include "halo.hpp"

namespace orc {

struct SellDev {
    int64_t n = 0;
    int64_t ncols = 0;
    int32_t n_slices = 0;
    int32_t ragged = 0;
    int64_t padded = 0;
    const int64_t *slice_ptr = nullptr;
    const int32_t *row_len = nullptr;
    const int32_t *col = nullptr;
    const int32_t *diag_pos = nullptr;
    const uint16_t *col16 = nullptr;
    const int32_t *colbase = nullptr;
    const long long *rows_base = nullptr;
    const int32_t *rows_intra = nullptr;
    const int32_t *rows_col = nullptr;
    const int64_t *csr_row_ptr = nullptr;
    int64_t nnz = 0;
};

struct PackedDev {
    const int64_t *ptr = nullptr;
    const int32_t *col = nullptr;
    const double *val = nullptr;
    int64_t total = 0;
};

constexpr int kXWinRows = 256;
constexpr int kXWinCap = 5000;
struct XWinDev {
    const int32_t *wcol = nullptr;
    const int32_t *wsize = nullptr;
    const uint16_t *lidx = nullptr;
    int32_t cap = kXWinCap;
    double *fold_scratch = nullptr;
    unsigned *fold_counter = nullptr;
};

struct RowsDev {
    const long long *slice_base = nullptr;
    const int32_t *intra_off = nullptr;
    const int32_t *col = nullptr;
    const double *val = nullptr;
};

struct MatView {
    SellDev P;
    const double *val = nullptr;
    const double *s1 = nullptr;
    const double *s2 = nullptr;
    int nt = 0;
    PackedDev pk;
    XWinDev xw;
    RowsDev rows;
    bool symmetric = true;
    bool persistent_pattern = false;
    HaloPlan *halo = nullptr;
    int32_t slice_lo = 0, slice_hi = -1, part_stride = 0, part_base = 0;
};

struct MatView3 {
    SellDev P;
    const double *val[3] = {nullptr, nullptr, nullptr};
    const double *s1 = nullptr, *s2 = nullptr;
    bool mesh_pattern = false;
    int nt = 0;
    HaloPlan *halo = nullptr;
    int32_t slice_lo = 0, slice_hi = -1, part_stride = 0, part_base = 0;
};

struct SellMatrix {
    int64_t n = 0, ncols = 0, nnz = 0, padded = 0;
    int32_t n_slices = 0;
    bool symmetric = true;
    int ragged = 0;
    DevBuf<int64_t> slice_ptr;
    DevBuf<int32_t> row_len, col, diag_pos, colbase;
    DevBuf<uint16_t> col16;
    DevBuf<int64_t> csr_row_ptr;
    DevBuf<long long> rows_base;
    DevBuf<int32_t> rows_intra, rows_col;
    SellDev dev() const {
        SellDev d;
        d.n = n; d.ncols = ncols; d.n_slices = n_slices; d.ragged = ragged; d.padded = padded; d.slice_ptr = slice_ptr.p; d.row_len = row_len.p; d.col = col.p; d.diag_pos = diag_pos.p;
        d.col16 = col16.p; d.colbase = colbase.p;
        d.rows_base = rows_base.p; d.rows_intra = rows_intra.p; d.rows_col = rows_col.p; d.csr_row_ptr = csr_row_ptr.p; d.nnz = nnz;
        return d;
    }
};

int sell_from_csr_host(int64_t n, int64_t ncols, const int64_t *row_ptr, const int64_t *col, SellMatrix &out);
int sell_import_values(const SellMatrix &m, const double *csr_vals_dev, double *sell_vals_dev);
int sell_export_values(const SellMatrix &m, const double *sell_vals_dev, double *csr_vals_dev);
int sell_rows_values_dev(const SellDev &P, const double *sell_vals_dev, double *rows_vals_dev);

struct SolveSide {
    hipStream_t stream = nullptr;
    Arena *arena = nullptr;
    hipEvent_t ev_setup = nullptr, ev_solve = nullptr;
};

struct AmgHierarchy {
    struct Level {
        int *choice = nullptr, *chooser = nullptr;
        SellDev P;
        double *val = nullptr;
        PackedDev pk;
        XWinDev xw;
        RowsDev rows;
        int64_t n = 0, padded = 0;
        int rounds = 0;
    } level[4];
    int n_levels = 0;
    int64_t n_fine = 0;
};

struct SiblingPairing {
    static constexpr int kLevels = 8;
    DevBuf<int> buf[kLevels];
    int64_t n[kLevels] = {0};
    hipEvent_t ready[kLevels] = {nullptr};
    bool published[kLevels] = {false};
    bool leader_done = true;
    std::mutex mu;
    std::condition_variable cv;
    ~SiblingPairing();
    void begin(bool leader_will_run);
    int publish(int level, const int *choice, int64_t rows, hipStream_t stream);
    const int *wait(int level, int64_t rows, hipStream_t stream);
    void finish();

    struct Offer {
        bool made = false, ok = false;
        const MatView *view = nullptr;
        Arena *arena = nullptr, *rows_arena = nullptr;
        hipEvent_t view_ready = nullptr;
        bool answered = false, adopted = false;
        void *level = nullptr;
    } offer[2];
    int expected_offers = 0;
    hipEvent_t ops_ready = nullptr;
    const int *lead_choice = nullptr, *lead_chooser = nullptr;
    void set_expected(int n);
    int make_offer(int slot, const MatView *view, Arena *arena, Arena *rows_arena, void *level, hipStream_t stream);
    void withdraw(int slot);
    bool wait_answer(int slot, hipStream_t stream);
    int collect_offers(Offer *out[2]);
    int answer(const bool adopted[2], const int *choice, const int *chooser, hipStream_t stream);
};

struct SolveStats {
    SiblingPairing *sibling = nullptr;
    int sibling_role = 0;
    SolveSide *side = nullptr;
    const AmgHierarchy *hierarchy = nullptr;
    int64_t jacobi_sweeps = 0;
    int64_t gmres_steps = 0, gmres_cycles = 0;
    double gmres_beta0 = 0., gmres_estimate = 0.;
    int amg_levels = 0;
    int64_t amg_rows[8] = {0};
    int64_t amg_nnz[8] = {0};
    int amg_rounds[8] = {0};
};

int iterative_solve_dev(const MatView &A, const double *b, double *x, uint64_t iteration_count, int method,
                        double relaxation_factor, double convergence_threshold, int preconditioner, Arena &arena,
                        SolveStats *stats);

int multigrid_prepare_dev(const MatView &A, int preconditioner, Arena &arena, AmgHierarchy &H, SiblingPairing *sibling = nullptr,
                          int sibling_role = 0, Arena *scratch = nullptr);
int diag_inverse_dev(const MatView &A, double *dinv);
int scale_vec_dev(const double *s, const double *b, double *out, int64_t n);
int multigrid_coarse_part_dev(const MatView &A, const double *r, double *x, uint64_t iteration_count, double relaxation_factor,
                              double convergence_threshold, int preconditioner, Arena &arena, SolveStats *stats, int *dev_status);

int spmv_dev(const MatView &A, const double *x, double *y);
int bench_bicgstab_dev(const MatView &A, const double *b, double *x, int reps, Arena &arena, float *ms);

int residual_dev(const MatView &A, const double *b, const double *x, double *r);
int residual_norm2_dev(const MatView &A, const double *b, const double *x, double *partials, double *out, double *r_scratch = nullptr);
int dot_reference(const double *a, const double *b, int64_t n, double *out, const double *skip_flags);
int sum_reference(const double *a, int64_t n, double *out);

int interleave3_dev(const double *a, const double *b, const double *c, double *out3, int64_t n);
int deinterleave3_dev(const double *in3, double *a, double *b, double *c, int64_t n);
int diag_inverse3_dev(const MatView3 &A, double *dinv3);
// ... 45 lines not shown
```

orc_amd/csrc/linalg_kernels.hpp:

```cpp
#pragma once
#include "linalg.hpp"

namespace orc {

__device__ __forceinline__ double view_value(const MatView &A, int64_t row, int64_t pos) {
    double v = A.val[pos];
    if (A.s1) v = A.s1[row] * v;
    if (A.s2) v = A.s2[row] * v;
    return v;
}

template <bool NT, class T>
__device__ __forceinline__ T ld_stream(const T *p) {
    if (NT) return __builtin_nontemporal_load(p);
    return *p;
}

__device__ __forceinline__ double fold_partials_block(const double *__restrict__ partials, int count, double *lds16 ) {
    const int lane = threadIdx.x & 63, w = threadIdx.x >> 6;
    double a[4], b[4];
#pragma unroll
    for (int p = 0; p < 4; ++p) {
        const int vt = (w + 4 * p) * 64 + lane;
        a[p] = vt < count ? partials[vt] : 0.;
        b[p] = vt + 1024 < count ? partials[vt + 1024] : 0.;
    }
    __syncthreads();
#pragma unroll
    for (int p = 0; p < 4; ++p) {
        const int vt = (w + 4 * p) * 64 + lane;
        double v = 0.;
        if (vt < count) v += a[p];
        if (vt + 1024 < count) v += b[p];
        v = wave_sum(v);
        if (lane == 0) lds16[w + 4 * p] = v;
    }
    __syncthreads();
    double r = 0.;
#pragma unroll
    for (int i = 0; i < 16; ++i) r += lds16[i];
    return r;
}

template <int NQ>
__device__ __forceinline__ void fold_partials_multi(const double *__restrict__ partials, int count, double *lds , double (&out)[NQ]) {
    const int lane = threadIdx.x & 63, w = threadIdx.x >> 6;
    double a[NQ][4], b[NQ][4];
#pragma unroll
    for (int q = 0; q < NQ; ++q) {
#pragma unroll
        for (int p = 0; p < 4; ++p) {
            const int vt = (w + 4 * p) * 64 + lane;
            a[q][p] = vt < count ? partials[(size_t)q * count + vt] : 0.;
            b[q][p] = vt + 1024 < count ? partials[(size_t)q * count + vt + 1024] : 0.;
        }
    }
    __syncthreads();
#pragma unroll
    for (int q = 0; q < NQ; ++q) {
#pragma unroll
        for (int p = 0; p < 4; ++p) {
            const int vt = (w + 4 * p) * 64 + lane;
            double v = 0.;
            if (vt < count) v += a[q][p];
            if (vt + 1024 < count) v += b[q][p];
            v = wave_sum(v);
            if (lane == 0) lds[q * 16 + w + 4 * p] = v;
        }
    }
    __syncthreads();
#pragma unroll
    for (int q = 0; q < NQ; ++q) {
        double r = 0.;
#pragma unroll
        for (int i = 0; i < 16; ++i) r += lds[q * 16 + i];
        out[q] = r;
    }
}

struct SliceWalk {
    int64_t begin, end, step;
    __device__ __forceinline__ SliceWalk(int32_t n_slices, int32_t first = 0) : SliceWalk(n_slices, first, (int)blockIdx.x, (int)gridDim.x) {}
    __device__ __forceinline__ SliceWalk(int32_t n_slices, int32_t first, int block, int grid) {
        const int waves = blockDim.x >> 6;
        const int wave = __builtin_amdgcn_readfirstlane((int)(threadIdx.x >> 6));
        if ((grid & 7) == 0 && grid >= 8) {
            const int xcd = block & 7, bl = block >> 3, nb = grid >> 3;
            const int64_t spx = ((int64_t)(n_slices - first) + 7) / 8;
            const int64_t lo = (int64_t)first + (int64_t)xcd * spx;
            int64_t hi = lo + spx;
            if (hi > n_slices) hi = n_slices;
            begin = lo + (int64_t)bl * waves + wave;
            end = hi;
            step = (int64_t)nb * waves;
        } else {
            begin = (int64_t)first + (int64_t)block * waves + wave;
            end = n_slices;
            step = (int64_t)grid * waves;
        }
    }
};

enum { kSpmvPlain = 0, kSpmvRagged = 1, kSpmvPacked = 2 };
template <class Epi, int kLayout = kSpmvPlain, bool kNoGather = false, bool kGuard = false>
__global__ __launch_bounds__(kBlock) void spmv_k(MatView A, const double *__restrict__ x, Epi epi, double *__restrict__ partials,
                                                 const double *__restrict__ skip_flags ) {
    __shared__ double lds[8];
    if (skip_flags && (skip_flags[0] != 0. || skip_flags[1] != 0.)) return;
    const int lane = threadIdx.x & 63;
    double r0 = 0., r1 = 0.;
    SliceWalk w(A.P.n_slices);
    for (int64_t slice = w.begin; slice < w.end; slice += w.step) {
        const int64_t row = slice * 64 + lane;
        const int64_t base = A.P.slice_ptr[slice];
        const int width = (int)((A.P.slice_ptr[slice + 1] - base) >> 6);
        const bool live = row < A.P.n;
        const int len = live ? A.P.row_len[row] : 0;
        const double s1 = (A.s1 && live) ? A.s1[row] : 1.;
        const double s2 = (A.s2 && live) ? A.s2[row] : 1.;
        double acc = 0.;
        int64_t pk_off = kLayout == kSpmvPacked ? A.pk.ptr[slice] : 0;
        const int last = (kLayout == kSpmvRagged ? (len > 0 ? len : 1) : width) - 1;
        const int lane_c = live ? lane : (int)((A.P.n - 1) & 63);
        for (int k0 = 0; k0 < width; k0 += 8) {
            int c[8];
            double v[8], xv[8];
#pragma unroll
            for (int u = 0; u < 8; ++u) {
                if (kLayout == kSpmvPacked) {
                    const bool in = k0 + u < len;
                    const unsigned long long m = __ballot(in);
                    const int rank = __builtin_amdgcn_mbcnt_hi((unsigned)(m >> 32), __builtin_amdgcn_mbcnt_lo((unsigned)m, 0u));
                    const int64_t p = in ? pk_off + rank : (m != 0ull ? pk_off : pk_off - 1);
                    c[u] = A.pk.col[p];
                    v[u] = A.pk.val[p];
                    pk_off += __popcll(m);
                } else if (kGuard) {
                    if (k0 + u < width) {
                        const int kk = kLayout == kSpmvPlain ? k0 + u : (k0 + u < last ? k0 + u : last);
                        const int64_t p = kLayout == kSpmvPlain ? (base + (int64_t)k0 * 64 + lane_c) + (int64_t)u * 64 : base + (int64_t)kk * 64 + lane_c;
                        c[u] = A.P.col[p];
                        v[u] = A.val[p];
                    } else { c[u] = 0; v[u] = 0.; }
                } else {
                    const int kk = k0 + u < last ? k0 + u : last;
                    const int64_t p = base + (int64_t)kk * 64 + lane_c;
                    c[u] = A.P.col[p];
                    v[u] = A.val[p];
                }
            }
#pragma unroll
            for (int u = 0; u < 8; ++u) {
                if (kGuard) { if (k0 + u < width) xv[u] = x[c[u]]; else xv[u] = 0.; }
                else xv[u] = x[kNoGather ? (int)(live ? row : 0) + (c[u] & 0) : c[u]];
            }
#pragma unroll
            for (int u = 0; u < 8; ++u) {
                double t = v[u];
                if (A.s1) t = s1 * t;
                if (A.s2) t = s2 * t;
                const double next = acc + t * xv[u];
                acc = (k0 + u < len) ? next : acc;
            }
        }
        if (live) epi.apply(row, acc, r0, r1);
    }
    if (Epi::kReductions > 0) {
        double t = block_sum(r0, lds);
        if (threadIdx.x == 0) partials[blockIdx.x] = t;
    }
    if (Epi::kReductions > 1) {
        double t = block_sum(r1, lds);
        if (threadIdx.x == 0) partials[gridDim.x + blockIdx.x] = t;
    }
}

template <class Epi, bool kRagged = false, bool kMesh = false, bool kNarrow = false, bool kScaled = true, bool kNT = false>
__global__ __launch_bounds__(kBlock) void spmv_uniform_k(MatView A, const double *__restrict__ x, Epi epi, double *__restrict__ partials,
                                                 const double *__restrict__ skip_flags ) {
    __shared__ double lds[8];
    if (skip_flags && (skip_flags[0] != 0. || skip_flags[1] != 0.)) return;
    const int lane = threadIdx.x & 63;
    double r0 = 0., r1 = 0.;
    SliceWalk w(A.slice_hi >= 0 ? A.slice_hi : A.P.n_slices, A.slice_lo);
    for (int64_t slice = w.begin; slice < w.end; slice += w.step) {
        const int64_t row = slice * 64 + lane;
        const int64_t base = A.P.slice_ptr[slice];
        const int width = (int)((A.P.slice_ptr[slice + 1] - base) >> 6);
        const bool live = row < A.P.n;
        const int len = live ? A.P.row_len[row] : 0;
        const double s1 = (kScaled && A.s1 && live) ? A.s1[row] : 1.;
        const double s2 = (kScaled && A.s2 && live) ? A.s2[row] : 1.;
        double acc = 0.;
        const int32_t *__restrict__ cb = kNarrow ? A.P.colbase + (base >> 6) : nullptr;
        for (int k0 = 0; k0 < width; k0 += 8) {
            int c[8];
            double v[8], xv[8];
            const int64_t p0 = base + (int64_t)k0 * 64 + lane;
            if (kNarrow) {
#pragma unroll
                for (int u = 0; u < 8; ++u) {
                    const bool in = k0 + u < width;
                    c[u] = in ? cb[k0 + u] + (int)ld_stream<kNT>(A.P.col16 + p0 + (int64_t)u * 64) : 0;
                    v[u] = in ? ld_stream<kNT>(A.val + p0 + (int64_t)u * 64) : 0.;
                }
            } else {
#pragma unroll
                for (int u = 0; u < 8; ++u) {
                    const bool in = k0 + u < (kRagged ? len : width);
                    c[u] = in ? ld_stream<kNT>(A.P.col + p0 + (int64_t)u * 64) : 0;
                    v[u] = in ? ld_stream<kNT>(A.val + p0 + (int64_t)u * 64) : 0.;
                }
            }
#pragma unroll
            for (int u = 0; u < 8; ++u) xv[u] = (k0 + u < len) ? x[c[u]] : 0.;
#pragma unroll
            for (int u = 0; u < 8; ++u) {
                if (k0 + u < len) {
                    double t = v[u];
                    if (kScaled && A.s1) t = s1 * t;
                    if (kScaled && A.s2) t = s2 * t;
                    acc += t * xv[u];
                }
            }
        }
        if (live) epi.apply(row, acc, r0, r1);
    }
    const int pstride = A.part_stride > 0 ? A.part_stride : (int)gridDim.x;
    if (Epi::kReductions > 0) {
        double t = block_sum(r0, lds);
        if (threadIdx.x == 0) partials[A.part_base + blockIdx.x] = t;
    }
    if (Epi::kReductions > 1) {
        double t = block_sum(r1, lds);
        if (threadIdx.x == 0) partials[pstride + A.part_base + blockIdx.x] = t;
    }
}


struct __attribute__((aligned(8))) Vec3d { double a, b, c; };

template <class Epi3, int kChunk = 4, bool kMesh = false, bool kNarrow = false, bool kScaled = true, bool kNT = false>
__global__ __launch_bounds__(kBlock) void spmv3_uniform_k(MatView3 A, const double *__restrict__ x3, Epi3 epi, double *__restrict__ partials) {
    __shared__ double lds[8];
    const int lane = threadIdx.x & 63;
    const Vec3d *__restrict__ xv3 = reinterpret_cast<const Vec3d *>(x3);
    const Vec3d *__restrict__ s1v = reinterpret_cast<const Vec3d *>(A.s1);
    const Vec3d *__restrict__ s2v = reinterpret_cast<const Vec3d *>(A.s2);
    const int vgrid = (int)gridDim.x;
    for (int vb = blockIdx.x; vb < vgrid; vb += gridDim.x) {
    double red[3][2] = {{0., 0.}, {0., 0.}, {0., 0.}};
    SliceWalk w(A.slice_hi >= 0 ? A.slice_hi : A.P.n_slices, A.slice_lo, vb, vgrid);
    for (int64_t slice = w.begin; slice < w.end; slice += w.step) {
        const int64_t row = slice * 64 + lane;
        const int64_t base = A.P.slice_ptr[slice];
        const int width = (int)((A.P.slice_ptr[slice + 1] - base) >> 6);
        const bool live = row < A.P.n;
        const int len = live ? A.P.row_len[row] : 0;
        Vec3d s1 = {1., 1., 1.}, s2 = {1., 1., 1.};
        if (kScaled && A.s1 && live) s1 = s1v[row];
        if (kScaled && A.s2 && live) s2 = s2v[row];
        double acc0 = 0., acc1 = 0., acc2 = 0.;
        const int32_t *__restrict__ cb = kNarrow ? A.P.colbase + (base >> 6) : nullptr;
        for (int k0 = 0; k0 < width; k0 += kChunk) {
            int c[kChunk];
            double v0[kChunk], v1[kChunk], v2[kChunk];
            Vec3d xv[kChunk];
            const int64_t p0 = base + (int64_t)k0 * 64 + lane;
#pragma unroll
            for (int u = 0; u < kChunk; ++u) {
                const bool in = k0 + u < width;
                if (kNarrow) c[u] = in ? cb[k0 + u] + (int)ld_stream<kNT>(A.P.col16 + p0 + (int64_t)u * 64) : 0;
                else c[u] = in ? ld_stream<kNT>(A.P.col + p0 + (int64_t)u * 64) : 0;
                v0[u] = in ? ld_stream<kNT>(A.val[0] + p0 + (int64_t)u * 64) : 0.;
                v1[u] = in ? ld_stream<kNT>(A.val[1] + p0 + (int64_t)u * 64) : 0.;
                v2[u] = in ? ld_stream<kNT>(A.val[2] + p0 + (int64_t)u * 64) : 0.;
            }
#pragma unroll
            for (int u = 0; u < kChunk; ++u) {
                if (k0 + u < len) xv[u] = xv3[c[u]];
                else xv[u] = Vec3d{0., 0., 0.};
            }
#pragma unroll
            for (int u = 0; u < kChunk; ++u) {
                if (k0 + u < len) {
                    double t0 = v0[u], t1 = v1[u], t2 = v2[u];
                    if (kScaled && A.s1) { t0 = s1.a * t0; t1 = s1.b * t1; t2 = s1.c * t2; }
                    if (kScaled && A.s2) { t0 = s2.a * t0; t1 = s2.b * t1; t2 = s2.c * t2; }
                    acc0 += t0 * xv[u].a;
                    acc1 += t1 * xv[u].b;
                    acc2 += t2 * xv[u].c;
                }
            }
        }
        if (live) {
            const double acc[3] = {acc0, acc1, acc2};
            epi.apply(row, acc, red);
        }
    }
#pragma unroll
    for (int s = 0; s < 3; ++s) {
#pragma unroll
        for (int q = 0; q < Epi3::kReductions; ++q) {
            const double t = block_sum(red[s][q], lds);
            if (threadIdx.x == 0) partials[(size_t)(s * Epi3::kReductions + q) * (A.part_stride > 0 ? A.part_stride : vgrid) + A.part_base + vb] = t;
        }
    }
    }
}

template <int kLayout>
struct SpmvSliceMeta {
    int64_t base, row, pk_off;
    int width, len, last;
    bool live;
    double s1, s2;
    int lane_c;
    __device__ __forceinline__ void load(const MatView &A, int64_t slice, int lane) {
        row = slice * 64 + lane;
        lane_c = row < A.P.n ? lane : (int)((A.P.n - 1) & 63);
        base = A.P.slice_ptr[slice];
        width = (int)((A.P.slice_ptr[slice + 1] - base) >> 6);
        live = row < A.P.n;
        len = live ? A.P.row_len[row] : 0;
        s1 = (A.s1 && live) ? A.s1[row] : 1.;
        s2 = (A.s2 && live) ? A.s2[row] : 1.;
        pk_off = kLayout == kSpmvPacked ? A.pk.ptr[slice] : 0;
        last = (kLayout == kSpmvRagged ? (len > 0 ? len : 1) : width) - 1;
    }
    __device__ __forceinline__ void issue(const MatView &A, int k0, int lane, int (&c)[8], double (&v)[8]) {
        if (width <= 0) {
#pragma unroll
            for (int u = 0; u < 8; ++u) { c[u] = 0; v[u] = 0.; }
            return;
        }
#pragma unroll
        for (int u = 0; u < 8; ++u) {
            if (kLayout == kSpmvPacked) {
                const bool in = k0 + u < len;
                const unsigned long long m = __ballot(in);
                const int rank = __builtin_amdgcn_mbcnt_hi((unsigned)(m >> 32), __builtin_amdgcn_mbcnt_lo((unsigned)m, 0u));
                const int64_t p = in ? pk_off + rank : (m != 0ull ? pk_off : pk_off - 1);
                c[u] = A.pk.col[p];
                v[u] = A.pk.val[p];
                pk_off += __popcll(m);
            } else {
                const int kk = k0 + u < last ? k0 + u : last;
                const int64_t p = base + (int64_t)kk * 64 + lane_c;
                c[u] = A.P.col[p];
                v[u] = A.val[p];
            }
        }
    }
};

template <class Epi, bool kScaled = true, bool kNT = false, int kC = 8>
__global__ __launch_bounds__(kBlock) void spmv_xwin_k(MatView A, const double *__restrict__ x, Epi epi, double *__restrict__ partials,
                                                      const double *__restrict__ skip_flags) {
    __shared__ double lds[8];
    extern __shared__ __align__(16) double xs[];
    if (skip_flags && (skip_flags[0] != 0. || skip_flags[1] != 0.)) return;
    const int lane = threadIdx.x & 63, wave = __builtin_amdgcn_readfirstlane((int)(threadIdx.x >> 6));
    double r0 = 0., r1 = 0.;
    const int64_t n_blocks = ((int64_t)A.P.n_slices + 3) >> 2;
    int64_t b_begin, b_end, b_step;
    if ((gridDim.x & 7) == 0 && gridDim.x >= 8) {
        const int xcd = blockIdx.x & 7, bl = blockIdx.x >> 3, nb = gridDim.x >> 3;
        const int64_t per = (n_blocks + 7) / 8;
        b_begin = (int64_t)xcd * per + bl;
        b_end = (int64_t)(xcd + 1) * per < n_blocks ? (int64_t)(xcd + 1) * per : n_blocks;
        b_step = nb;
    } else {
        b_begin = blockIdx.x; b_end = n_blocks; b_step = gridDim.x;
    }
    for (int64_t b = b_begin; b < b_end; b += b_step) {
        const int ws_built = A.xw.wsize[b];
        const int ws = ws_built <= A.xw.cap ? ws_built : -1;
        const int64_t slice = b * 4 + wave;
        const bool has_slice = slice < A.P.n_slices;
        const int64_t row = slice * 64 + lane;
        const bool live = has_slice && row < A.P.n;
        int width = 0, len = 0;
        int64_t pk_off = 0;
        if (has_slice) {
            const int64_t base = A.P.slice_ptr[slice];
            width = (int)((A.P.slice_ptr[slice + 1] - base) >> 6);
            len = live ? A.P.row_len[row] : 0;
            pk_off = A.pk.ptr[slice];
        }
        const int64_t sb = __builtin_amdgcn_readfirstlane((int)(pk_off & 0xffffffff)) | ((int64_t)__builtin_amdgcn_readfirstlane((int)(pk_off >> 32)) << 32);
        const unsigned short *s_lidx = A.xw.lidx + sb;
        const double *s_val = A.pk.val + sb;
        int off32 = 0;
        int c[kC], cn[kC];
        double v[kC], vn[kC];
        auto issue = [&](int k0, int (&cc)[kC], double (&vv)[kC]) {
#pragma unroll
            for (int u = 0; u < kC; ++u) {
                const bool in = k0 + u < len;
                const unsigned long long m = __ballot(in);
                const int rank = __builtin_amdgcn_mbcnt_hi((unsigned)(m >> 32), __builtin_amdgcn_mbcnt_lo((unsigned)m, 0u));
                const int p = in ? off32 + rank : (m != 0ull ? off32 : off32 - 1);
                cc[u] = (int)ld_stream<kNT>(s_lidx + p);
                vv[u] = ld_stream<kNT>(s_val + p);
                off32 += __popcll(m);
            }
        };
        if (ws > 0) {
            const int32_t *wc = A.xw.wcol + b * kXWinCap;
            for (int j0 = 0; j0 < ws; j0 += 8 * kBlock) {
                int wj[8];
                double xw[8];
#pragma unroll
                for (int q = 0; q < 8; ++q) {
                    const int j = j0 + q * kBlock + (int)threadIdx.x;
                    wj[q] = ld_stream<kNT>(wc + (j < ws ? j : 0));
                }
#pragma unroll
                for (int q = 0; q < 8; ++q) xw[q] = x[wj[q]];
#pragma unroll
                for (int q = 0; q < 8; ++q) {
                    const int j = j0 + q * kBlock + (int)threadIdx.x;
                    if (j < ws) xs[j] = xw[q];
                }
            }
        }
        __syncthreads();
        if (has_slice) {
            const double s1 = (kScaled && A.s1 && live) ? A.s1[row] : 1.;
            const double s2 = (kScaled && A.s2 && live) ? A.s2[row] : 1.;
            double acc = 0.;
            if (ws >= 0) {
                auto consume = [&](int k0, const int (&cc)[kC], const double (&vv)[kC]) {
                    double xv[kC];
#pragma unroll
                    for (int u = 0; u < kC; ++u) xv[u] = xs[cc[u]];
#pragma unroll
                    for (int u = 0; u < kC; ++u) {
                        double t = vv[u];
                        if (kScaled && A.s1) t = s1 * t;
                        if (kScaled && A.s2) t = s2 * t;
                        const double next = acc + t * xv[u];
                        acc = (k0 + u < len) ? next : acc;
                    }
                };
                if (width > 0) issue(0, c, v);
                int k0 = 0;
                for (; k0 + kC < width; k0 += 2 * kC) {
                    issue(k0 + kC, cn, vn);
                    consume(k0, c, v);
                    if (k0 + 2 * kC < width) issue(k0 + 2 * kC, c, v);
                    consume(k0 + kC, cn, vn);
                }
                if (k0 < width) consume(k0, c, v);
            } else {
                for (int k0 = 0; k0 < width; k0 += 8) {
                    int cg[8];
                    double vg[8], xv[8];
#pragma unroll
                    for (int u = 0; u < 8; ++u) {
                        const bool in = k0 + u < len;
                        const unsigned long long m = __ballot(in);
                        const int rank = __builtin_amdgcn_mbcnt_hi((unsigned)(m >> 32), __builtin_amdgcn_mbcnt_lo((unsigned)m, 0u));
                        const int64_t p = in ? pk_off + rank : (m != 0ull ? pk_off : pk_off - 1);
                        cg[u] = ld_stream<kNT>(A.pk.col + p);
                        vg[u] = ld_stream<kNT>(A.pk.val + p);
                        pk_off += __popcll(m);
                    }
#pragma unroll
                    for (int u = 0; u < 8; ++u) xv[u] = x[cg[u]];
#pragma unroll
                    for (int u = 0; u < 8; ++u) {
                        double t = vg[u];
                        if (kScaled && A.s1) t = s1 * t;
                        if (kScaled && A.s2) t = s2 * t;
                        const double next = acc + t * xv[u];
                        acc = (k0 + u < len) ? next : acc;
                    }
                }
            }
            if (live) epi.apply(row, acc, r0, r1);
        }
        __syncthreads();
    }
    if (Epi::kReductions > 0 && A.xw.fold_scratch) {
        __shared__ int s_last;
        const int nwg = (int)gridDim.x;
        const double t0 = block_sum(r0, lds);
        const double t1 = Epi::kReductions > 1 ? block_sum(r1, lds) : 0.;
        if (threadIdx.x == 0) {
            __hip_atomic_store(A.xw.fold_scratch + blockIdx.x, t0, __ATOMIC_RELAXED, __HIP_MEMORY_SCOPE_AGENT);
            if (Epi::kReductions > 1) __hip_atomic_store(A.xw.fold_scratch + nwg + blockIdx.x, t1, __ATOMIC_RELAXED, __HIP_MEMORY_SCOPE_AGENT);
            __builtin_amdgcn_s_waitcnt(0);
            s_last = __hip_atomic_fetch_add(A.xw.fold_counter, 1u, __ATOMIC_RELAXED, __HIP_MEMORY_SCOPE_AGENT) == (unsigned)(nwg - 1);
        }
        __syncthreads();
        if (s_last) {
            const double *fs = A.xw.fold_scratch;
#pragma unroll
            for (int q = 0; q < Epi::kReductions; ++q) {
                double v = 0.;
                for (int i0 = threadIdx.x; i0 < nwg; i0 += 8 * kBlock) {
                    double t[8];
#pragma unroll
                    for (int u = 0; u < 8; ++u) {
                        const int i = i0 + u * kBlock;
                        t[u] = i < nwg ? __hip_atomic_load(fs + (size_t)q * nwg + i, __ATOMIC_RELAXED, __HIP_MEMORY_SCOPE_AGENT) : 0.;
                    }
#pragma unroll
                    for (int u = 0; u < 8; ++u) v += t[u];
                }
                v = block_sum(v, lds);
                if (threadIdx.x == 0) partials[q] = v;
            }
            if (threadIdx.x == 0) __hip_atomic_store(A.xw.fold_counter, 0u, __ATOMIC_RELAXED, __HIP_MEMORY_SCOPE_AGENT);
        }
        return;
    }
    if (Epi::kReductions > 0) {
        double t = block_sum(r0, lds);
        if (threadIdx.x == 0) partials[blockIdx.x] = t;
    }
    if (Epi::kReductions > 1) {
        double t = block_sum(r1, lds);
        if (threadIdx.x == 0) partials[gridDim.x + blockIdx.x] = t;
    }
}

__global__ __launch_bounds__(1024) void reduce_partials_k(const double *__restrict__ partials, int count, int nq, double *__restrict__ out);

int reduce_partials(const double *partials, int count, int nq, double *out, bool global = false);

}
```

orc_amd/linear_algebra.py:

```python
import ctypes as C

import numpy as np

from ._lib import check, lib


def _i64(a):
    return np.ascontiguousarray(a, dtype=np.int64)


def _f64(a):
    return np.ascontiguousarray(a, dtype=np.float64)


def _p(a, t):
    return a.ctypes.data_as(C.POINTER(t))


def iterative_solve(a, b, solution_vector, iteration_count, method, relaxation_factor, convergence_threshold,
                    preconditioner, raise_on_error=True):
    a = a.tocsr()
    a.sort_indices()
    rp, ci, v = _i64(a.indptr), _i64(a.indices), _f64(a.data)
    b = _f64(b)
    assert solution_vector.dtype == np.float64 and solution_vector.flags.c_contiguous
    st = lib().orc_iterative_solve(C.c_int64(a.shape[0]), _p(rp, C.c_int64), _p(ci, C.c_int64), _p(v, C.c_double),
                                   _p(b, C.c_double), _p(solution_vector, C.c_double), C.c_uint64(iteration_count),
                                   C.c_int(method), C.c_double(relaxation_factor), C.c_double(convergence_threshold),
                                   C.c_int(preconditioner))
    if raise_on_error:
        check(st)
    return st


def iterative_solve3(a_list, b_list, x_list, iteration_count, method, relaxation_factor, convergence_threshold, preconditioner):
    a0 = a_list[0]
    n = a0.shape[0]
    rp, ci = _i64(a0.indptr), _i64(a0.indices)
    for a in a_list[1:]:
        assert np.array_equal(a.indptr, a0.indptr) and np.array_equal(a.indices, a0.indices), "the three systems must share their pattern"
    vals = [_f64(a.data) for a in a_list]
    bs = [_f64(b) for b in b_list]
    for x in x_list:
        assert x.dtype == np.float64 and x.flags.c_contiguous and len(x) == n
    PD = C.POINTER(C.c_double)
    v3 = (PD * 3)(*[_p(v, C.c_double) for v in vals])
    b3 = (PD * 3)(*[_p(b, C.c_double) for b in bs])
    x3 = (PD * 3)(*[_p(x, C.c_double) for x in x_list])
    st3 = (C.c_int * 3)()
    st = lib().orc_iterative_solve3(C.c_int64(n), _p(rp, C.c_int64), _p(ci, C.c_int64), v3, b3, x3, C.c_uint64(iteration_count), C.c_int(method),
                                    C.c_double(relaxation_factor), C.c_double(convergence_threshold), C.c_int(preconditioner), st3)
    return st, [st3[0], st3[1], st3[2]]


def set_breakdown_guard(on):
    check(lib().orc_set_breakdown_guard(C.c_int(1 if on else 0)))


def set_reduction_order(order):
    check(lib().orc_set_reduction_order(C.c_int(int(order))))


def breakdown_guard_events(reset=False):
    lib().orc_breakdown_guard_events.restype = C.c_int64
    return int(lib().orc_breakdown_guard_events(C.c_int(1 if reset else 0)))


def last_jacobi_sweeps():
    return lib().orc_last_jacobi_sweeps()


def set_gmres_restart(m):
    check(lib().orc_set_gmres_restart(C.c_int(int(m))))


def last_gmres_stats():
    steps, cycles = C.c_int64(0), C.c_int64(0)
    beta0, est = C.c_double(0.0), C.c_double(0.0)
    check(lib().orc_last_gmres_stats(C.byref(steps), C.byref(cycles), C.byref(beta0), C.byref(est)))
    return steps.value, cycles.value, beta0.value, est.value


def csr_spmv(a, x, reps=1):
    a = a.tocsr()
    a.sort_indices()
    rp, ci, v = _i64(a.indptr), _i64(a.indices), _f64(a.data)
    x = _f64(x)
    y = np.empty(a.shape[0])
    ms = C.c_double(0.0)
    check(lib().orc_csr_spmv(C.c_int64(a.shape[0]), _p(rp, C.c_int64), _p(ci, C.c_int64), _p(v, C.c_double),
                             _p(x, C.c_double), _p(y, C.c_double), C.c_int(reps), C.byref(ms)))
    return y, ms.value


def amg_coarsen(a):
    import scipy.sparse as sp
    a = a.tocsr()
    a.sort_indices()
    n = a.shape[0]
    rp, ci, v = _i64(a.indptr), _i64(a.indices), _f64(a.data)
    partner = np.empty(n, np.int64)
    nc, nnz, rounds = C.c_int64(0), C.c_int64(0), C.c_int(0)
    args = (C.c_int64(n), _p(rp, C.c_int64), _p(ci, C.c_int64), _p(v, C.c_double), _p(partner, C.c_int64), C.byref(nc), C.byref(nnz))
    check(lib().orc_amg_coarsen(*args, None, None, None, C.byref(rounds)))
    orp, oci, ov = np.empty(nc.value + 1, np.int64), np.empty(nnz.value, np.int64), np.empty(nnz.value)
    check(lib().orc_amg_coarsen(*args, _p(orp, C.c_int64), _p(oci, C.c_int64), _p(ov, C.c_double), C.byref(rounds)))
    return partner, sp.csr_matrix((ov, oci, orp), shape=(nc.value, nc.value)), rounds.value


def debug_coloring(a):
    a = a.tocsr()
    a.sort_indices()
    n = a.shape[0]
    rp, ci = _i64(a.indptr), _i64(a.indices)
    colors = np.empty(n, np.int32)
    nc = C.c_int32(0)
    check(lib().orc_debug_coloring(C.c_int64(n), _p(rp, C.c_int64), _p(ci, C.c_int64), _p(colors, C.c_int32), C.byref(nc)))
    return colors, nc.value


def amg_coarse_product(a, x, scaled=False):
    a = a.tocsr()
    a.sort_indices()
    n = a.shape[0]
    rp, ci, v = _i64(a.indptr), _i64(a.indices), _f64(a.data)
    x = _f64(x)
    assert len(x) == (n + 1) // 2
    y = np.empty(len(x))
    mirror = C.c_int(0)
    check(lib().orc_debug_amg_coarse_product(C.c_int64(n), _p(rp, C.c_int64), _p(ci, C.c_int64), _p(v, C.c_double), C.c_int(1 if scaled else 0),
                                             _p(x, C.c_double), _p(y, C.c_double), C.byref(mirror)))
    return y, bool(mirror.value)


def xwin_counters(reset=False):
    out = (C.c_longlong * 3)()
    check(lib().orc_debug_xwin_counters(out, C.c_int(1 if reset else 0)))
    return out[0], out[1], out[2]


def shared_galerkin(reset=False):
    f = lib().orc_debug_shared_galerkin
    f.restype = C.c_longlong
    return int(f(C.c_int(1 if reset else 0)))


def amg_certification(reset=False):
    out = (C.c_longlong * 2)()
    check(lib().orc_debug_amg_certification(out, C.c_int(1 if reset else 0)))
    return out[0], out[1]
```

Before: 1.355.

## Pack AMG coarse-level mirror in pairs and chunked window indices for vector loads

Changes the packed mirror layout of coarse AMG matrices so that values and columns are stored in per-row pairs. Window-local column indices are stored in chunks of kPackChunk 16-bit entries per lane, with a separate offset table (lptr). The SpMV kernels now issue one ballot per pair or chunk and read them with 128-bit and 64-bit vector loads, instead of one ballot and one scalar load per nonzero. This cuts per-element index arithmetic and memory transactions, at the cost of padding storage for odd row lengths and chunk tails, plus an extra scan and offset table. A debug export entry point is also added.

```diff
diff --git a/include/orc_amd.h b/include/orc_amd.h
--- a/include/orc_amd.h
+++ b/include/orc_amd.h
@@ -161,6 +161,8 @@
 int orc_debug_stream_report(char *buf, int cap);
 int orc_debug_amg_coarse_product(int64_t n, const int64_t *row_ptr, const int64_t *col_idx, const double *values, int scaled, const double *x,
                                  double *y, int *has_window_mirror);
+int orc_debug_amg_packed_mirror(int64_t n, const int64_t *row_ptr, const int64_t *col_idx, const double *values, int64_t sizes[5], int32_t *row_len,
+                                int64_t *pk_ptr, int32_t *pk_col, double *pk_val, int64_t *lptr, uint16_t *lidx, int32_t *wcol, int32_t *wsize);
 long long orc_debug_collectives(int reset);
 int orc_debug_clamp_partials_grid(long long requested);
 int orc_debug_max_partials(void);
diff --git a/orc_amd/csrc/amg.hip b/orc_amd/csrc/amg.hip
--- a/orc_amd/csrc/amg.hip
+++ b/orc_amd/csrc/amg.hip
@@ -537,25 +537,32 @@
             }
             __syncthreads();
             const int kend = min(kPackDepth, width - kc);
-            for (int q = 0; q < kend; ++q) {
+            const int kend_pk = pk_ptr ? min(kPackDepth, ((width + 1) & ~1) - kc) : kend;
+            int pair_rank = 0;
+            int64_t pair_base = 0;
+            for (int q = 0; q < kend_pk; ++q) {
                 const int k = kc + q;
                 const bool in = k < len;
                 const int c = (in && !kValuesOnly) ? t_col[q * 65 + lane] : (int)I;
                 const double v = in ? t_val[q * 65 + lane] : 0.;
-                const int64_t pos = base + (int64_t)k * 64 + lane;
-                if (live) {
+                if (live && q < kend) {
+                    const int64_t pos = base + (int64_t)k * 64 + lane;
                     if (!kValuesOnly) col_c[pos] = c;
                     val_c[pos] = v;
                     if (!kValuesOnly && in && c == (int)I) d = (int)pos;
                 }
                 if (pk_ptr) {
-                    const unsigned long long m = __ballot(in);
-                    const int rank = __builtin_amdgcn_mbcnt_hi((unsigned)(m >> 32), __builtin_amdgcn_mbcnt_lo((unsigned)m, 0u));
-                    if (in) {
-                        if (!kValuesOnly) pk_col[pk_off + rank] = c;
-                        pk_val[pk_off + rank] = v;
+                    if ((k & 1) == 0) {
+                        const unsigned long long m = __ballot(in);
+                        pair_rank = __builtin_amdgcn_mbcnt_hi((unsigned)(m >> 32), __builtin_amdgcn_mbcnt_lo((unsigned)m, 0u));
+                        pair_base = pk_off;
+                        pk_off += 2 * (int64_t)__popcll(m);
                     }
-                    pk_off += __popcll(m);
+                    if ((k & ~1) < len) {
+                        const int64_t p = pair_base + 2 * pair_rank + (k & 1);
+                        if (!kValuesOnly) pk_col[p] = c;
+                        pk_val[p] = v;
+                    }
                 }
             }
             __syncthreads();
@@ -651,19 +658,26 @@
 }
 
 __global__ __launch_bounds__(kBlock) void slice_sizes_k(const int *__restrict__ row_len, int64_t n, int n_slices, int64_t *__restrict__ w_sell,
-                                                        int64_t *__restrict__ w_pk) {
+                                                        int64_t *__restrict__ w_pk, int64_t *__restrict__ w_pos, int64_t *__restrict__ w_tot) {
     const int lane = threadIdx.x & 63;
     const int64_t wave = ((int64_t)blockIdx.x * blockDim.x + threadIdx.x) >> 6, waves = ((int64_t)gridDim.x * blockDim.x) >> 6;
     for (int64_t s = wave; s < n_slices; s += waves) {
         const int64_t r = s * 64 + lane;
         const int len = r < n ? row_len[r] : 0;
-        int mx = len, sum = len;
+        int mx = len, sum = len, pairs = (len + 1) >> 1, chunks = (len + kPackChunk - 1) / kPackChunk;
 #pragma unroll
         for (int off = 32; off > 0; off >>= 1) {
             mx = max(mx, __shfl_xor(mx, off, 64));
             sum += __shfl_xor(sum, off, 64);
-        }
-        if (lane == 0) { w_sell[s] = (int64_t)mx * 64; w_pk[s] = ((int64_t)sum + 15) & ~(int64_t)15; }
+            pairs += __shfl_xor(pairs, off, 64);
+            chunks += __shfl_xor(chunks, off, 64);
+        }
+        if (lane == 0) {
+            w_sell[s] = (int64_t)mx * 64;
+            w_pk[s] = ((int64_t)pairs * 2 + 15) & ~(int64_t)15;
+            w_pos[s] = ((int64_t)chunks * kPackChunk + 63) & ~(int64_t)63;
+            w_tot[s] = ((int64_t)sum + 15) & ~(int64_t)15;
+        }
     }
 }
 constexpr int kScanBlocks = 128;
@@ -724,7 +738,7 @@
 __device__ unsigned long long g_xwin_counters[3];
 constexpr int kXBitWordsSmall = 4096;
 template <int kWords, bool kSecond>
-__global__ __launch_bounds__(kBlock) void xwin_build_k(SellDev P, PackedDev pk, int *__restrict__ wcol, int *__restrict__ wsize,
+__global__ __launch_bounds__(kBlock) void xwin_build_k(SellDev P, const int64_t *__restrict__ lptr, int *__restrict__ wcol, int *__restrict__ wsize,
                                                        unsigned short *__restrict__ lidx, int64_t n_blocks, int win_cap, int bit_words, int pass_words,
                                                        int *__restrict__ pending ) {
     if (kSecond && *pending == 0) return;
@@ -808,16 +822,24 @@
         if (slice < P.n_slices) {
             const int64_t sbase = P.slice_ptr[slice];
             const int width = (int)((P.slice_ptr[slice + 1] - sbase) >> 6);
-            int64_t off = pk.ptr[slice];
-            for (int q = 0; q < width; ++q) {
-                const bool in = q < len;
+            int64_t off = lptr[slice];
+            for (int j0 = 0; j0 < width; j0 += kPackChunk) {
+                const bool in = j0 < len;
                 const unsigned long long m = __ballot(in);
                 const int rank = __builtin_amdgcn_mbcnt_hi((unsigned)(m >> 32), __builtin_amdgcn_mbcnt_lo((unsigned)m, 0u));
                 if (in) {
-                    const int c = P.col[sbase + (int64_t)q * 64 + lane] - cmin;
-                    lidx[off + rank] = (unsigned short)(wpre[c >> 5] + __popc(bits[c >> 5] & ((1u << (c & 31)) - 1u)));
+                    u32x4_t w = {0u, 0u, 0u, 0u};
+#pragma unroll
+                    for (int u = 0; u < kPackChunk; ++u) {
+                        if (j0 + u < len) {
+                            const int c = P.col[sbase + (int64_t)(j0 + u) * 64 + lane] - cmin;
+                            const unsigned pos = wpre[c >> 5] + __popc(bits[c >> 5] & ((1u << (c & 31)) - 1u));
+                            w[u >> 1] |= pos << (16 * (u & 1));
+                        }
+                    }
+                    *reinterpret_cast<u32x4_t *>(lidx + off + (int64_t)kPackChunk * rank) = w;
                 }
-                off += __popcll(m);
+                off += (int64_t)kPackChunk * __popcll(m);
             }
         }
         __syncthreads();
@@ -1555,17 +1577,26 @@
 #undef ORC_MERGE
     }
     lap("galerkin product");
-    int64_t *pk_ptr, *w_sell, *w_pk;
+    int64_t *pk_ptr, *lptr, *w_sell, *w_pk, *w_pos, *w_tot, *tot_ptr;
     ORC_TRY(arena.alloc((size_t)n_slices + 1, &pk_ptr));
+    ORC_TRY(arena.alloc((size_t)n_slices + 1, &lptr));
     ORC_TRY(tmp.alloc((size_t)n_slices + 1, &w_sell));
     ORC_TRY(tmp.alloc((size_t)n_slices + 1, &w_pk));
-    hipLaunchKernelGGL(slice_sizes_k, dim3((unsigned)std::min<int64_t>(((int64_t)n_slices + 3) / 4, 4096)), dim3(kBlock), 0, st, row_len, nc, n_slices, w_sell, w_pk);
+    ORC_TRY(tmp.alloc((size_t)n_slices + 1, &w_pos));
+    ORC_TRY(tmp.alloc((size_t)n_slices + 1, &w_tot));
+    ORC_TRY(arena.alloc((size_t)n_slices + 1, &tot_ptr));
+    hipLaunchKernelGGL(slice_sizes_k, dim3((unsigned)std::min<int64_t>(((int64_t)n_slices + 3) / 4, 4096)), dim3(kBlock), 0, st, row_len, nc, n_slices, w_sell, w_pk,
+                       w_pos, w_tot);
     static_assert(sizeof(long long) == sizeof(int64_t), "64-bit tables");
     ORC_TRY(scan_excl_dev(reinterpret_cast<const long long *>(w_sell), reinterpret_cast<const long long *>(w_pk), (int64_t)n_slices, reinterpret_cast<long long *>(slice_ptr),
                           reinterpret_cast<long long *>(pk_ptr), true, scan_part, st));
+    ORC_TRY(scan_excl_dev(reinterpret_cast<const long long *>(w_pos), reinterpret_cast<const long long *>(w_tot), (int64_t)n_slices, reinterpret_cast<long long *>(lptr),
+                          reinterpret_cast<long long *>(tot_ptr), true, scan_part, st));
     ORC_HIP(hipGetLastError());
-    int64_t padded = 0, packed_total = 0;
-    ORC_HIP(hipMemcpyAsync(&packed_total, pk_ptr + n_slices, sizeof(int64_t), hipMemcpyDeviceToHost, st));
+    int64_t padded = 0, packed_total = 0, packed_slots = 0, pos_slots = 0;
+    ORC_HIP(hipMemcpyAsync(&packed_total, tot_ptr + n_slices, sizeof(int64_t), hipMemcpyDeviceToHost, st));
+    ORC_HIP(hipMemcpyAsync(&packed_slots, pk_ptr + n_slices, sizeof(int64_t), hipMemcpyDeviceToHost, st));
+    ORC_HIP(hipMemcpyAsync(&pos_slots, lptr + n_slices, sizeof(int64_t), hipMemcpyDeviceToHost, st));
     ORC_HIP(hipMemcpyAsync(&padded, slice_ptr + n_slices, sizeof(int64_t), hipMemcpyDeviceToHost, st));
     ORC_HIP(hipMemcpyAsync(hflags, flags, sizeof(hflags), hipMemcpyDeviceToHost, st));
     ORC_HIP(hipStreamSynchronize(st));
@@ -1584,8 +1615,8 @@
     int *pk_col = nullptr;
     double *pk_val = nullptr;
     if (mirror) {
-        ORC_TRY(arena.alloc((size_t)packed_total, &pk_col));
-        ORC_TRY(arena.alloc((size_t)packed_total, &pk_val));
+        ORC_TRY(arena.alloc((size_t)packed_slots, &pk_col));
+        ORC_TRY(arena.alloc((size_t)packed_slots, &pk_val));
     }
     hipLaunchKernelGGL(galerkin_pack_fused_k<false>, dim3((unsigned)std::max<int64_t>(1, std::min<int64_t>(n_slices, 256 * 12))), dim3(64), 0, st, Pc, slice_base, intra_off,
                        s_col, s_val, col, val, diag, mirror ? (const int64_t *)pk_ptr : (const int64_t *)nullptr, pk_col, pk_val);
@@ -1593,7 +1624,7 @@
     double *x_val[2] = {nullptr, nullptr}, *x_pk_val[2] = {nullptr, nullptr};
     for (int x = 0; x < n_sib; ++x) {
         ORC_TRY(sib[x].arena->alloc((size_t)std::max<int64_t>(padded, 1), &x_val[x]));
-        if (mirror) ORC_TRY(sib[x].arena->alloc((size_t)packed_total, &x_pk_val[x]));
+        if (mirror) ORC_TRY(sib[x].arena->alloc((size_t)packed_slots, &x_pk_val[x]));
         hipLaunchKernelGGL(galerkin_pack_fused_k<true>, dim3((unsigned)std::max<int64_t>(1, std::min<int64_t>(n_slices, 256 * 12))), dim3(64), 0, st, Pc, slice_base, intra_off,
                            s_col, (const double *)X.s_val[x], (int *)nullptr, x_val[x], (int *)nullptr, mirror ? (const int64_t *)pk_ptr : (const int64_t *)nullptr, (int *)nullptr,
                            x_pk_val[x]);
@@ -1636,9 +1667,9 @@
         ORC_TRY(rows_arena.alloc(ncs, &r_intra));
         L.rows_transient = true;
         hipLaunchKernelGGL(rows_compact_k, dim3((unsigned)std::max<int64_t>(1, std::min<int64_t>(n_slices, 256 * 16))), dim3(64), 0, st, (const int *)row_len, nc, n_slices,
-                           (const long long *)slice_base, (const int *)intra_off, (const int *)s_col, (const double *)s_val, (const int64_t *)pk_ptr, r_intra, r_col, r_val);
+                           (const long long *)slice_base, (const int *)intra_off, (const int *)s_col, (const double *)s_val, (const int64_t *)tot_ptr, r_intra, r_col, r_val);
         ORC_HIP(hipGetLastError());
-        L.rows.slice_base = reinterpret_cast<const long long *>(pk_ptr); L.rows.intra_off = r_intra; L.rows.col = r_col; L.rows.val = r_val;
+        L.rows.slice_base = reinterpret_cast<const long long *>(tot_ptr); L.rows.intra_off = r_intra; L.rows.col = r_col; L.rows.val = r_val;
         for (int x = 0; x < n_sib; ++x) {
             Arena &xa = sib[x].rows_arena ? *sib[x].rows_arena : *sib[x].arena;
             if (sib[x].rows_arena) xa.release(Arena::Mark{0, 0});
@@ -1648,31 +1679,31 @@
             ORC_TRY(xa.alloc((size_t)packed_total, &xr_val));
             ORC_TRY(xa.alloc(ncs, &xr_intra));
             hipLaunchKernelGGL(rows_compact_k, dim3((unsigned)std::max<int64_t>(1, std::min<int64_t>(n_slices, 256 * 16))), dim3(64), 0, st, (const int *)row_len, nc, n_slices,
-                               (const long long *)slice_base, (const int *)intra_off, (const int *)s_col, (const double *)X.s_val[x], (const int64_t *)pk_ptr, xr_intra, xr_col, xr_val);
+                               (const long long *)slice_base, (const int *)intra_off, (const int *)s_col, (const double *)X.s_val[x], (const int64_t *)tot_ptr, xr_intra, xr_col, xr_val);
             ORC_HIP(hipGetLastError());
             CoarseLevel &Lx = *sib[x].L;
-            Lx.rows.slice_base = reinterpret_cast<const long long *>(pk_ptr); Lx.rows.intra_off = xr_intra; Lx.rows.col = xr_col; Lx.rows.val = xr_val;
+            Lx.rows.slice_base = reinterpret_cast<const long long *>(tot_ptr); Lx.rows.intra_off = xr_intra; Lx.rows.col = xr_col; Lx.rows.val = xr_val;
             Lx.rows_transient = sib[x].rows_arena != nullptr;
         }
     }
     if (mirror) {
-        L.pk.ptr = pk_ptr; L.pk.col = pk_col; L.pk.val = pk_val; L.pk.total = packed_total;
+        L.pk.ptr = pk_ptr; L.pk.col = pk_col; L.pk.val = pk_val; L.pk.total = packed_total; L.pk.slots = packed_slots;
         const int64_t n_blocks = ((int64_t)n_slices + 3) / 4;
         int *wcol, *wsize;
         unsigned short *lidx;
         ORC_TRY(arena.alloc((size_t)n_blocks * kXWinCap, &wcol));
         ORC_TRY(arena.alloc((size_t)n_blocks, &wsize));
-        ORC_TRY(arena.alloc((size_t)packed_total, &lidx));
+        ORC_TRY(arena.alloc((size_t)std::max<int64_t>(pos_slots, 1), &lidx));
         const int win_cap = cfg().xwin_cap > 0 ? std::min(kXWinCap, cfg().xwin_cap) : kXWinCap;
         const int bit_words = cfg().xwin_bitwords > 0 ? std::min(kXBitWords, cfg().xwin_bitwords) : kXBitWords;
         const int small_words = cfg().xwin_small_bitwords > 0 ? std::min(kXBitWordsSmall, cfg().xwin_small_bitwords) : kXBitWordsSmall;
         int *pending;
         ORC_TRY(tmp.alloc((size_t)1, &pending));
         ORC_HIP(hipMemsetAsync(pending, 0, sizeof(int), st));
-        hipLaunchKernelGGL(HIP_KERNEL_NAME(xwin_build_k<kXBitWordsSmall, false>), dim3((unsigned)std::min<int64_t>(n_blocks, 2048)), dim3(kBlock), 0, st, Pc, L.pk, wcol, wsize, lidx,
+        hipLaunchKernelGGL(HIP_KERNEL_NAME(xwin_build_k<kXBitWordsSmall, false>), dim3((unsigned)std::min<int64_t>(n_blocks, 2048)), dim3(kBlock), 0, st, Pc, (const int64_t *)lptr, wcol, wsize, lidx,
                            n_blocks, win_cap, bit_words, small_words, pending);
         if (bit_words > small_words)
-            hipLaunchKernelGGL(HIP_KERNEL_NAME(xwin_build_k<kXBitWords, true>), dim3((unsigned)std::min<int64_t>(n_blocks, 2048)), dim3(kBlock), 0, st, Pc, L.pk, wcol, wsize, lidx,
+            hipLaunchKernelGGL(HIP_KERNEL_NAME(xwin_build_k<kXBitWords, true>), dim3((unsigned)std::min<int64_t>(n_blocks, 2048)), dim3(kBlock), 0, st, Pc, (const int64_t *)lptr, wcol, wsize, lidx,
                                n_blocks, win_cap, bit_words, kXBitWords, pending);
         if (trace_t) {
             int hp = 0;
@@ -1681,7 +1712,7 @@
             fprintf(stderr, "[amg windows n=%lld] %lld blocks, %d left to the full bitmap\n", (long long)nc, (long long)n_blocks, hp);
         }
         ORC_HIP(hipGetLastError());
-        L.xw.wcol = wcol; L.xw.wsize = wsize; L.xw.lidx = lidx;
+        L.xw.wcol = wcol; L.xw.wsize = wsize; L.xw.lidx = lidx; L.xw.lptr = lptr;
         {
             int *over;
             ORC_TRY(tmp.alloc((size_t)kXWinCapSizes, &over));
@@ -2336,4 +2367,35 @@
     return ORC_OK;
 }
 
-}
+int amg_debug_packed(const MatView &A, Arena &arena, int64_t sizes[5], int32_t *row_len_h, int64_t *pk_ptr_h, int32_t *pk_col_h, double *pk_val_h,
+                     int64_t *lptr_h, uint16_t *lidx_h, int32_t *wcol_h, int32_t *wsize_h) {
+    hipStream_t st = ctx().stream;
+    Arena::Mark mk = arena.mark();
+    int *choice, *chooser;
+    const int64_t n = A.P.n;
+    ORC_TRY(arena.alloc((size_t)std::max<int64_t>(n, 1), &choice));
+    ORC_TRY(arena.alloc((size_t)std::max<int64_t>(n, 1), &chooser));
+    CoarseLevel L;
+    ORC_TRY(aggregate(A, arena, choice, chooser, &L.rounds));
+    ORC_TRY(galerkin(A, choice, chooser, arena, L));
+    const bool mirror = L.pk.ptr && L.xw.lidx;
+    const int64_t ns = L.P.n_slices, nb = (ns + 3) / 4;
+    sizes[0] = L.n; sizes[1] = ns; sizes[2] = mirror ? L.pk.slots : 0; sizes[3] = 0; sizes[4] = mirror ? nb : 0;
+    if (mirror) ORC_HIP(hipMemcpyAsync(&sizes[3], L.xw.lptr + ns, sizeof(int64_t), hipMemcpyDeviceToHost, st));
+    ORC_HIP(hipStreamSynchronize(st));
+    if (mirror && row_len_h && pk_ptr_h && pk_col_h && pk_val_h && lptr_h && lidx_h && wcol_h && wsize_h) {
+        ORC_HIP(hipMemcpyAsync(row_len_h, L.P.row_len, sizeof(int32_t) * (size_t)L.n, hipMemcpyDeviceToHost, st));
+        ORC_HIP(hipMemcpyAsync(pk_ptr_h, L.pk.ptr, sizeof(int64_t) * (size_t)(ns + 1), hipMemcpyDeviceToHost, st));
+        ORC_HIP(hipMemcpyAsync(pk_col_h, L.pk.col, sizeof(int32_t) * (size_t)sizes[2], hipMemcpyDeviceToHost, st));
+        ORC_HIP(hipMemcpyAsync(pk_val_h, L.pk.val, sizeof(double) * (size_t)sizes[2], hipMemcpyDeviceToHost, st));
+        ORC_HIP(hipMemcpyAsync(lptr_h, L.xw.lptr, sizeof(int64_t) * (size_t)(ns + 1), hipMemcpyDeviceToHost, st));
+        ORC_HIP(hipMemcpyAsync(lidx_h, L.xw.lidx, sizeof(uint16_t) * (size_t)sizes[3], hipMemcpyDeviceToHost, st));
+        ORC_HIP(hipMemcpyAsync(wcol_h, L.xw.wcol, sizeof(int32_t) * (size_t)(nb * kXWinCap), hipMemcpyDeviceToHost, st));
+        ORC_HIP(hipMemcpyAsync(wsize_h, L.xw.wsize, sizeof(int32_t) * (size_t)nb, hipMemcpyDeviceToHost, st));
+        ORC_HIP(hipStreamSynchronize(st));
+    }
+    arena.release(mk);
+    return ORC_OK;
+}
+
+}
diff --git a/orc_amd/csrc/api_linalg.cpp b/orc_amd/csrc/api_linalg.cpp
--- a/orc_amd/csrc/api_linalg.cpp
+++ b/orc_amd/csrc/api_linalg.cpp
@@ -6,6 +6,8 @@
 int amg_debug_coarsen(const MatView &A, Arena &arena, std::vector<int> &choice_h, std::vector<int64_t> &row_ptr_h,
                       std::vector<int64_t> &col_h, std::vector<double> &val_h, int *rounds, const double *x_h = nullptr, double *y_h = nullptr,
                       int scaled = 0, int *mirror_out = nullptr);
+int amg_debug_packed(const MatView &A, Arena &arena, int64_t sizes[5], int32_t *row_len_h, int64_t *pk_ptr_h, int32_t *pk_col_h, double *pk_val_h,
+                     int64_t *lptr_h, uint16_t *lidx_h, int32_t *wcol_h, int32_t *wsize_h);
 int gs_debug_coloring(const SellDev &P, std::vector<int> &colors, int *n_colors);
 static SolveStats g_last_stats;
 SolveStats &last_stats() { return g_last_stats; }
@@ -206,6 +208,25 @@
     return amg_debug_coarsen(A, arena, choice, rp, ci, v, nullptr, x, y, scaled, has_window_mirror);
 }
 
+int orc_debug_amg_packed_mirror(int64_t n, const int64_t *row_ptr, const int64_t *col_idx, const double *values, int64_t sizes[5], int32_t *row_len,
+                                int64_t *pk_ptr, int32_t *pk_col, double *pk_val, int64_t *lptr, uint16_t *lidx, int32_t *wcol, int32_t *wsize) {
+    using namespace orc;
+    ORC_TRY(ensure_init());
+    if (n < 1 || !row_ptr || !col_idx || !values || !sizes) return set_error(ORC_ERR_BAD_ARGUMENT, "null argument");
+    SellMatrix pat;
+    ORC_TRY(sell_from_csr_host(n, n, row_ptr, col_idx, pat));
+    DevBuf<double> csr_vals, vals;
+    ORC_TRY(csr_vals.upload(values, (size_t)pat.nnz));
+    ORC_TRY(vals.alloc((size_t)std::max<int64_t>(pat.padded, 1)));
+    ORC_TRY(sell_import_values(pat, csr_vals.p, vals.p));
+    MatView A;
+    A.P = pat.dev();
+    A.val = vals.p;
+    A.symmetric = pat.symmetric;
+    Arena arena;
+    return amg_debug_packed(A, arena, sizes, row_len, pk_ptr, pk_col, pk_val, lptr, lidx, wcol, wsize);
+}
+
 int orc_debug_coloring(int64_t n, const int64_t *row_ptr, const int64_t *col_idx, int32_t *colors, int32_t *n_colors) {
     using namespace orc;
     ORC_TRY(ensure_init());
diff --git a/orc_amd/csrc/linalg.hip b/orc_amd/csrc/linalg.hip
--- a/orc_amd/csrc/linalg.hip
+++ b/orc_amd/csrc/linalg.hip
@@ -712,16 +712,18 @@
         const int len = live ? A.P.row_len[row] : 0;
         const double s1 = (A.s1 && live) ? A.s1[row] : 1.;
         const double s2 = (A.s2 && live) ? A.s2[row] : 1.;
-        int64_t off = A.pk.ptr[slice];
-        for (int k = 0; k < width; ++k) {
+        const f64x2_t *src = reinterpret_cast<const f64x2_t *>(A.pk.val + A.pk.ptr[slice]);
+        f64x2_t *dst = reinterpret_cast<f64x2_t *>(out + A.pk.ptr[slice]);
+        int off = 0;
+        for (int k = 0; k < width; k += 2) {
             const bool in = k < len;
             const unsigned long long m = __ballot(in);
             const int rank = __builtin_amdgcn_mbcnt_hi((unsigned)(m >> 32), __builtin_amdgcn_mbcnt_lo((unsigned)m, 0u));
             if (in) {
-                double t = A.pk.val[off + rank];
-                if (A.s1) t = s1 * t;
-                if (A.s2) t = s2 * t;
-                out[off + rank] = t;
+                f64x2_t t = src[off + rank];
+                if (A.s1) { t.x = s1 * t.x; t.y = s1 * t.y; }
+                if (A.s2) { t.x = s2 * t.x; t.y = s2 * t.y; }
+                dst[off + rank] = t;
             }
             off += __popcll(m);
         }
@@ -733,7 +735,7 @@
     if (A.pk.ptr) {
         if (!(A.xw.lidx && A.pk.total > 0)) return ORC_OK;
         double *scaled;
-        ORC_TRY(arena.alloc((size_t)A.pk.total, &scaled));
+        ORC_TRY(arena.alloc((size_t)A.pk.slots, &scaled));
         hipLaunchKernelGGL(scale_packed_k, dim3(spmv_grid(A.P.n_slices)), dim3(kBlock), 0, ctx().stream, A, scaled);
         ORC_HIP(hipGetLastError());
         A.pk.val = scaled;
diff --git a/orc_amd/csrc/linalg.hpp b/orc_amd/csrc/linalg.hpp
--- a/orc_amd/csrc/linalg.hpp
+++ b/orc_amd/csrc/linalg.hpp
@@ -26,11 +26,13 @@
     int64_t nnz = 0;
 };
 
+constexpr int kPackChunk = 8;
 struct PackedDev {
     const int64_t *ptr = nullptr;
     const int32_t *col = nullptr;
     const double *val = nullptr;
     int64_t total = 0;
+    int64_t slots = 0;
 };
 
 constexpr int kXWinRows = 256;
@@ -39,6 +41,7 @@
     const int32_t *wcol = nullptr;
     const int32_t *wsize = nullptr;
     const uint16_t *lidx = nullptr;
+    const int64_t *lptr = nullptr;
     int32_t cap = kXWinCap;
     double *fold_scratch = nullptr;
     unsigned *fold_counter = nullptr;
diff --git a/orc_amd/csrc/linalg_kernels.hpp b/orc_amd/csrc/linalg_kernels.hpp
--- a/orc_amd/csrc/linalg_kernels.hpp
+++ b/orc_amd/csrc/linalg_kernels.hpp
@@ -14,6 +14,18 @@
 __device__ __forceinline__ T ld_stream(const T *p) {
     if (NT) return __builtin_nontemporal_load(p);
     return *p;
+}
+
+typedef unsigned u32x4_t __attribute__((ext_vector_type(4)));
+typedef int i32x2_t __attribute__((ext_vector_type(2)));
+typedef double f64x2_t __attribute__((ext_vector_type(2)));
+
+__device__ __forceinline__ int packed_pair(bool in, int &off) {
+    const unsigned long long m = __ballot(in);
+    const int rank = __builtin_amdgcn_mbcnt_hi((unsigned)(m >> 32), __builtin_amdgcn_mbcnt_lo((unsigned)m, 0u));
+    const int p = in ? off + rank : (m != 0ull ? off : off - 1);
+    off += __popcll(m);
+    return p;
 }
 
 __device__ __forceinline__ double fold_partials_block(const double *__restrict__ partials, int count, double *lds16 ) {
@@ -119,34 +131,39 @@
         const double s1 = (A.s1 && live) ? A.s1[row] : 1.;
         const double s2 = (A.s2 && live) ? A.s2[row] : 1.;
         double acc = 0.;
-        int64_t pk_off = kLayout == kSpmvPacked ? A.pk.ptr[slice] : 0;
+        const i32x2_t *pk_c = kLayout == kSpmvPacked ? reinterpret_cast<const i32x2_t *>(A.pk.col + A.pk.ptr[slice]) : nullptr;
+        const f64x2_t *pk_v = kLayout == kSpmvPacked ? reinterpret_cast<const f64x2_t *>(A.pk.val + A.pk.ptr[slice]) : nullptr;
+        int pk_off = 0;
         const int last = (kLayout == kSpmvRagged ? (len > 0 ? len : 1) : width) - 1;
         const int lane_c = live ? lane : (int)((A.P.n - 1) & 63);
         for (int k0 = 0; k0 < width; k0 += 8) {
             int c[8];
             double v[8], xv[8];
-#pragma unroll
-            for (int u = 0; u < 8; ++u) {
-                if (kLayout == kSpmvPacked) {
-                    const bool in = k0 + u < len;
-                    const unsigned long long m = __ballot(in);
-                    const int rank = __builtin_amdgcn_mbcnt_hi((unsigned)(m >> 32), __builtin_amdgcn_mbcnt_lo((unsigned)m, 0u));
-                    const int64_t p = in ? pk_off + rank : (m != 0ull ? pk_off : pk_off - 1);
-                    c[u] = A.pk.col[p];
-                    v[u] = A.pk.val[p];
-                    pk_off += __popcll(m);
-                } else if (kGuard) {
-                    if (k0 + u < width) {
-                        const int kk = kLayout == kSpmvPlain ? k0 + u : (k0 + u < last ? k0 + u : last);
-                        const int64_t p = kLayout == kSpmvPlain ? (base + (int64_t)k0 * 64 + lane_c) + (int64_t)u * 64 : base + (int64_t)kk * 64 + lane_c;
+            if (kLayout == kSpmvPacked) {
+#pragma unroll
+                for (int q = 0; q < 4; ++q) {
+                    const int p = packed_pair(k0 + 2 * q < len, pk_off);
+                    const i32x2_t cc = pk_c[p];
+                    const f64x2_t vv = pk_v[p];
+                    c[2 * q] = cc.x; c[2 * q + 1] = cc.y;
+                    v[2 * q] = vv.x; v[2 * q + 1] = vv.y;
+                }
+            } else {
+#pragma unroll
+                for (int u = 0; u < 8; ++u) {
+                    if (kGuard) {
+                        if (k0 + u < width) {
+                            const int kk = kLayout == kSpmvPlain ? k0 + u : (k0 + u < last ? k0 + u : last);
+                            const int64_t p = kLayout == kSpmvPlain ? (base + (int64_t)k0 * 64 + lane_c) + (int64_t)u * 64 : base + (int64_t)kk * 64 + lane_c;
+                            c[u] = A.P.col[p];
+                            v[u] = A.val[p];
+                        } else { c[u] = 0; v[u] = 0.; }
+                    } else {
+                        const int kk = k0 + u < last ? k0 + u : last;
+                        const int64_t p = base + (int64_t)kk * 64 + lane_c;
                         c[u] = A.P.col[p];
                         v[u] = A.val[p];
-                    } else { c[u] = 0; v[u] = 0.; }
-                } else {
-                    const int kk = k0 + u < last ? k0 + u : last;
-                    const int64_t p = base + (int64_t)kk * 64 + lane_c;
-                    c[u] = A.P.col[p];
-                    v[u] = A.val[p];
+                    }
                 }
             }
 #pragma unroll
@@ -309,56 +326,12 @@
     }
 }
 
-template <int kLayout>
-struct SpmvSliceMeta {
-    int64_t base, row, pk_off;
-    int width, len, last;
-    bool live;
-    double s1, s2;
-    int lane_c;
-    __device__ __forceinline__ void load(const MatView &A, int64_t slice, int lane) {
-        row = slice * 64 + lane;
-        lane_c = row < A.P.n ? lane : (int)((A.P.n - 1) & 63);
-        base = A.P.slice_ptr[slice];
-        width = (int)((A.P.slice_ptr[slice + 1] - base) >> 6);
-        live = row < A.P.n;
-        len = live ? A.P.row_len[row] : 0;
-        s1 = (A.s1 && live) ? A.s1[row] : 1.;
-        s2 = (A.s2 && live) ? A.s2[row] : 1.;
-        pk_off = kLayout == kSpmvPacked ? A.pk.ptr[slice] : 0;
-        last = (kLayout == kSpmvRagged ? (len > 0 ? len : 1) : width) - 1;
-    }
-    __device__ __forceinline__ void issue(const MatView &A, int k0, int lane, int (&c)[8], double (&v)[8]) {
-        if (width <= 0) {
-#pragma unroll
-            for (int u = 0; u < 8; ++u) { c[u] = 0; v[u] = 0.; }
-            return;
-        }
-#pragma unroll
-        for (int u = 0; u < 8; ++u) {
-            if (kLayout == kSpmvPacked) {
-                const bool in = k0 + u < len;
-                const unsigned long long m = __ballot(in);
-                const int rank = __builtin_amdgcn_mbcnt_hi((unsigned)(m >> 32), __builtin_amdgcn_mbcnt_lo((unsigned)m, 0u));
-                const int64_t p = in ? pk_off + rank : (m != 0ull ? pk_off : pk_off - 1);
-                c[u] = A.pk.col[p];
-                v[u] = A.pk.val[p];
-                pk_off += __popcll(m);
-            } else {
-                const int kk = k0 + u < last ? k0 + u : last;
-                const int64_t p = base + (int64_t)kk * 64 + lane_c;
-                c[u] = A.P.col[p];
-                v[u] = A.val[p];
-            }
-        }
-    }
-};
-
-template <class Epi, bool kScaled = true, bool kNT = false, int kC = 8>
+template <class Epi, bool kScaled = true, bool kNT = false>
 __global__ __launch_bounds__(kBlock) void spmv_xwin_k(MatView A, const double *__restrict__ x, Epi epi, double *__restrict__ partials,
                                                       const double *__restrict__ skip_flags) {
     __shared__ double lds[8];
     extern __shared__ __align__(16) double xs[];
+    constexpr int kC = kPackChunk;
     if (skip_flags && (skip_flags[0] != 0. || skip_flags[1] != 0.)) return;
     const int lane = threadIdx.x & 63, wave = __builtin_amdgcn_readfirstlane((int)(threadIdx.x >> 6));
     double r0 = 0., r1 = 0.;
@@ -381,30 +354,30 @@
         const int64_t row = slice * 64 + lane;
         const bool live = has_slice && row < A.P.n;
         int width = 0, len = 0;
-        int64_t pk_off = 0;
+        int64_t pk_off = 0, lp_off = 0;
         if (has_slice) {
             const int64_t base = A.P.slice_ptr[slice];
             width = (int)((A.P.slice_ptr[slice + 1] - base) >> 6);
             len = live ? A.P.row_len[row] : 0;
             pk_off = A.pk.ptr[slice];
+            lp_off = ws >= 0 ? A.xw.lptr[slice] : 0;
         }
         const int64_t sb = __builtin_amdgcn_readfirstlane((int)(pk_off & 0xffffffff)) | ((int64_t)__builtin_amdgcn_readfirstlane((int)(pk_off >> 32)) << 32);
-        const unsigned short *s_lidx = A.xw.lidx + sb;
-        const double *s_val = A.pk.val + sb;
-        int off32 = 0;
-        int c[kC], cn[kC];
-        double v[kC], vn[kC];
-        auto issue = [&](int k0, int (&cc)[kC], double (&vv)[kC]) {
-#pragma unroll
-            for (int u = 0; u < kC; ++u) {
-                const bool in = k0 + u < len;
-                const unsigned long long m = __ballot(in);
+        const int64_t lb = __builtin_amdgcn_readfirstlane((int)(lp_off & 0xffffffff)) | ((int64_t)__builtin_amdgcn_readfirstlane((int)(lp_off >> 32)) << 32);
+        const u32x4_t *s_pos = reinterpret_cast<const u32x4_t *>(A.xw.lidx + lb);
+        const f64x2_t *s_val = reinterpret_cast<const f64x2_t *>(A.pk.val + sb);
+        int poff = 0, voff = 0;
+        u32x4_t c, cn;
+        f64x2_t v[kC / 2], vn[kC / 2];
+        auto issue = [&](int k0, u32x4_t &cc, f64x2_t (&vv)[kC / 2]) {
+            {
+                const unsigned long long m = __ballot(k0 < len);
                 const int rank = __builtin_amdgcn_mbcnt_hi((unsigned)(m >> 32), __builtin_amdgcn_mbcnt_lo((unsigned)m, 0u));
-                const int p = in ? off32 + rank : (m != 0ull ? off32 : off32 - 1);
-                cc[u] = (int)ld_stream<kNT>(s_lidx + p);
-                vv[u] = ld_stream<kNT>(s_val + p);
-                off32 += __popcll(m);
-            }
+                cc = ld_stream<kNT>(s_pos + poff + (k0 < len ? rank : 0));
+                poff += __popcll(m);
+            }
+#pragma unroll
+            for (int q = 0; q < kC / 2; ++q) vv[q] = ld_stream<kNT>(s_val + packed_pair(k0 + 2 * q < len, voff));
         };
         if (ws > 0) {
             const int32_t *wc = A.xw.wcol + b * kXWinCap;
@@ -431,13 +404,17 @@
             const double s2 = (kScaled && A.s2 && live) ? A.s2[row] : 1.;
             double acc = 0.;
             if (ws >= 0) {
-                auto consume = [&](int k0, const int (&cc)[kC], const double (&vv)[kC]) {
+                auto consume = [&](int k0, const u32x4_t &cc, const f64x2_t (&vv)[kC / 2]) {
                     double xv[kC];
 #pragma unroll
-                    for (int u = 0; u < kC; ++u) xv[u] = xs[cc[u]];
+                    for (int q = 0; q < kC / 2; ++q) {
+                        const unsigned w = cc[q];
+                        xv[2 * q] = xs[w & 0xffffu];
+                        xv[2 * q + 1] = xs[w >> 16];
+                    }
 #pragma unroll
                     for (int u = 0; u < kC; ++u) {
-                        double t = vv[u];
+                        double t = vv[u >> 1][u & 1];
                         if (kScaled && A.s1) t = s1 * t;
                         if (kScaled && A.s2) t = s2 * t;
                         const double next = acc + t * xv[u];
@@ -454,18 +431,17 @@
                 }
                 if (k0 < width) consume(k0, c, v);
             } else {
+                const i32x2_t *s_col = reinterpret_cast<const i32x2_t *>(A.pk.col + sb);
                 for (int k0 = 0; k0 < width; k0 += 8) {
                     int cg[8];
                     double vg[8], xv[8];
 #pragma unroll
-                    for (int u = 0; u < 8; ++u) {
-                        const bool in = k0 + u < len;
-                        const unsigned long long m = __ballot(in);
-                        const int rank = __builtin_amdgcn_mbcnt_hi((unsigned)(m >> 32), __builtin_amdgcn_mbcnt_lo((unsigned)m, 0u));
-                        const int64_t p = in ? pk_off + rank : (m != 0ull ? pk_off : pk_off - 1);
-                        cg[u] = ld_stream<kNT>(A.pk.col + p);
-                        vg[u] = ld_stream<kNT>(A.pk.val + p);
-                        pk_off += __popcll(m);
+                    for (int q = 0; q < 4; ++q) {
+                        const int p = packed_pair(k0 + 2 * q < len, voff);
+                        const i32x2_t cc = ld_stream<kNT>(s_col + p);
+                        const f64x2_t vv = ld_stream<kNT>(s_val + p);
+                        cg[2 * q] = cc.x; cg[2 * q + 1] = cc.y;
+                        vg[2 * q] = vv.x; vg[2 * q + 1] = vv.y;
                     }
 #pragma unroll
                     for (int u = 0; u < 8; ++u) xv[u] = x[cg[u]];
diff --git a/orc_amd/linear_algebra.py b/orc_amd/linear_algebra.py
--- a/orc_amd/linear_algebra.py
+++ b/orc_amd/linear_algebra.py
@@ -133,6 +133,26 @@
     return y, bool(mirror.value)
 
 
+def amg_packed_mirror(a):
+    a = a.tocsr()
+    a.sort_indices()
+    n = a.shape[0]
+    rp, ci, v = _i64(a.indptr), _i64(a.indices), _f64(a.data)
+    sizes = np.zeros(5, np.int64)
+    f = lib().orc_debug_amg_packed_mirror
+    null = [None] * 8
+    check(f(C.c_int64(n), _p(rp, C.c_int64), _p(ci, C.c_int64), _p(v, C.c_double), _p(sizes, C.c_int64), *null))
+    nc, ns, slots, pos_slots, nb = (int(t) for t in sizes)
+    if slots == 0:
+        return None
+    out = dict(row_len=np.empty(nc, np.int32), pk_ptr=np.empty(ns + 1, np.int64), pk_col=np.empty(slots, np.int32), pk_val=np.empty(slots),
+               lptr=np.empty(ns + 1, np.int64), lidx=np.empty(pos_slots, np.uint16), wcol=np.empty((nb, 5000), np.int32), wsize=np.empty(nb, np.int32))
+    check(f(C.c_int64(n), _p(rp, C.c_int64), _p(ci, C.c_int64), _p(v, C.c_double), _p(sizes, C.c_int64), _p(out["row_len"], C.c_int32),
+            _p(out["pk_ptr"], C.c_int64), _p(out["pk_col"], C.c_int32), _p(out["pk_val"], C.c_double), _p(out["lptr"], C.c_int64),
+            _p(out["lidx"], C.c_uint16), _p(out["wcol"], C.c_int32), _p(out["wsize"], C.c_int32)))
+    return out
+
+
 def xwin_counters(reset=False):
     out = (C.c_longlong * 3)()
     check(lib().orc_debug_xwin_counters(out, C.c_int(1 if reset else 0)))
```

Result: faster. 1.407, median of 6 (+3.8%).
